# sssxyd/cpp-paddle-ocr

Measured on AMD Instinct MI355X. Metric: images/sec end-to-end (det+cls+rec) at 960x960, higher is better.
Workload: dtype f32

## Files before the change

### cpp-paddle-ocr_amd/binding.py

```python
import ctypes as C
import os

import numpy as np

HERE = os.path.dirname(os.path.abspath(__file__))
ROOT = os.path.dirname(HERE)
LIB_PATH = os.environ.get("OCR_LIB_PATH") or os.path.join(HERE, "lib", "libocr_hip.so")
MODELS = os.path.join(ROOT, "models")

_lib = None


class OcrError(RuntimeError):
    pass


class ocr_img(C.Structure):
    _fields_ = [("data", C.c_void_p), ("rows", C.c_int), ("cols", C.c_int), ("row_stride", C.c_size_t)]


class ocr_det_cfg(C.Structure):
    _fields_ = [("model_dir", C.c_char_p), ("device_id", C.c_int), ("limit_type", C.c_char_p),
                ("limit_side_len", C.c_int), ("det_db_thresh", C.c_double), ("det_db_box_thresh", C.c_double),
                ("det_db_unclip_ratio", C.c_double), ("det_db_score_mode", C.c_char_p), ("use_dilation", C.c_int),
# ... 778 lines not shown
            self.h = None


class Cls:
    def __init__(self, model_dir=None, device=0, cls_thresh=0.98, cls_batch_num=8, precision="fp32"):
        L = lib()
        _stage_protos(L)
        cfg = ocr_cls_cfg()
        L.ocr_cls_cfg_default(C.byref(cfg))
        self._keep = [(model_dir or os.path.join(MODELS, "cls")).encode(), precision.encode()]
        cfg.model_dir, cfg.precision = self._keep
        cfg.device_id, cfg.cls_thresh, cfg.cls_batch_num = device, cls_thresh, cls_batch_num
        self.h = C.c_void_p()
        check(L.ocr_cls_create(C.byref(cfg), C.byref(self.h)))
        self.times = (C.c_double * 3)()

    def run(self, crops):
        n = len(crops)
        labels = np.zeros(n, np.int32)
        scores = np.zeros(n, np.float32)
        if n:
            check(lib().ocr_cls_run(self.h, _imgs(crops), n, labels.ctypes.data, scores.ctypes.data, self.times))
        return labels, scores

    def probs(self, n):
        out = np.empty((n, 2), np.float32)
        check(lib().ocr_cls_probs(self.h, out.ctypes.data, out.size))
        return out

    def close(self):
        if self.h:
            lib().ocr_cls_destroy(self.h)
            self.h = None


class Rec:
    def __init__(self, model_dir=None, device=0, label_path=None, rec_batch_num=16, rec_img_h=28, rec_img_w=192,
                 precision="fp32", sort_mode=0):
        L = lib()
        _stage_protos(L)
        cfg = ocr_rec_cfg()
        L.ocr_rec_cfg_default(C.byref(cfg))
        md = model_dir or os.path.join(MODELS, "rec")
        self._keep = [md.encode(), (label_path or os.path.join(md, "ppocr_keys_v1.txt")).encode(), precision.encode()]
        cfg.model_dir, cfg.label_path, cfg.precision = self._keep
        cfg.device_id, cfg.rec_batch_num, cfg.rec_img_h, cfg.rec_img_w = device, rec_batch_num, rec_img_h, rec_img_w
        cfg.sort_mode = int(sort_mode)
        self.h = C.c_void_p()
        check(L.ocr_rec_create(C.byref(cfg), C.byref(self.h)))
        self.times = (C.c_double * 3)()

    def run(self, crops, max_len=512):
        n = len(crops)
        ids = np.zeros((n, max_len), np.int32)
        lens = np.zeros(n, np.int32)
        scores = np.zeros(n, np.float32)
        if n:
            check(lib().ocr_rec_run(self.h, _imgs(crops), n, ids.ctypes.data, max_len, lens.ctypes.data,
                                    scores.ctypes.data, self.times))
        return [ids[i, :lens[i]].copy() for i in range(n)], scores

    def run_chars(self, crops, max_len=512, topk=0):
        n = len(crops)
        ids = np.zeros((n, max_len), np.int32)
        lens = np.zeros(n, np.int32)
        scores = np.zeros(n, np.float32)
        steps = np.zeros((n, max_len), np.int32)
        nsteps = np.zeros((n, max_len), np.int32)
        probs = np.zeros((n, max_len), np.float32)
        geom = np.zeros((n, 3), np.int32)
        kk = max(int(topk), 1)
        alt_ids = np.zeros((n, max_len, kk), np.int32)
        alt_probs = np.zeros((n, max_len, kk), np.float32)
        if n:
            check(lib().ocr_rec_run_chars(self.h, _imgs(crops), n, ids.ctypes.data, max_len, lens.ctypes.data, scores.ctypes.data,
                                          steps.ctypes.data, nsteps.ctypes.data, probs.ctypes.data, geom.ctypes.data, int(topk),
                                          alt_ids.ctypes.data, alt_probs.ctypes.data, self.times))
        chars = []
        for i in range(n):
            m = lens[i]
            c = dict(steps=steps[i, :m].copy(), nsteps=nsteps[i, :m].copy(), probs=probs[i, :m].copy(), geom=tuple(int(v) for v in geom[i]))
            if topk > 0:
                c["alt_ids"] = alt_ids[i, :m].copy()
                c["alt_probs"] = alt_probs[i, :m].copy()
            chars.append(c)
        return [ids[i, :lens[i]].copy() for i in range(n)], scores, chars

    def logits_row(self, index, step):
        out = np.zeros(self.num_classes(), np.float32)
        check(lib().ocr_rec_logits_row(self.h, int(index), int(step), out.ctypes.data, out.size))
        return out

    def steps(self, index, cap=4096):
        amax = np.zeros(cap, np.int32)
        pmax = np.zeros(cap, np.float32)
        T = C.c_int()
        check(lib().ocr_rec_steps(self.h, index, amax.ctypes.data, pmax.ctypes.data, cap, C.byref(T)))
        return amax[:T.value].copy(), pmax[:T.value].copy()

    def set_launch_lines(self, n):
        check(lib().ocr_rec_set_launch_lines(self.h, int(n)))

    def timing(self, on=True):
        check(lib().ocr_rec_timing(self.h, int(on)))

    def timing_report(self):
        buf = C.create_string_buffer(1 << 20)
        check(lib().ocr_rec_timing_report(self.h, buf, len(buf)))
        out = {}
        for line in buf.value.decode().splitlines():
            name, ms, cnt, fl, by = line.split()
            out[name] = dict(ms=float(ms), count=int(cnt), flops=float(fl), bytes=float(by))
        return out

    def label(self, i):
        s = lib().ocr_rec_label(self.h, int(i))
        return s.decode("utf-8") if s is not None else None

    def text(self, ids):
        return "".join(self.label(i) for i in ids)

    def num_classes(self):
        return lib().ocr_rec_num_classes(self.h)

    def close(self):
        if self.h:
            lib().ocr_rec_destroy(self.h)
            self.h = None


class ocr_pipe_cfg(C.Structure):
    _fields_ = [("det", ocr_det_cfg), ("cls", ocr_cls_cfg), ("rec", ocr_rec_cfg), ("enable_cls", C.c_int),
                ("crop_mode", C.c_int), ("phases", C.c_int)]


class ocr_word(C.Structure):
    _fields_ = [("box", C.c_int32 * 8), ("ids_off", C.c_int32), ("ids_len", C.c_int32), ("confidence", C.c_float)]


class ocr_char(C.Structure):
    _fields_ = [("step", C.c_int32), ("nsteps", C.c_int32), ("prob", C.c_float), ("quad", C.c_int32 * 8)]


EXPORTS += ["ocr_pipe_cfg_default", "ocr_pipe_create", "ocr_pipe_destroy", "ocr_pipe_run", "ocr_pipe_run_chars", "ocr_pipe_run_device",
            "ocr_pipe_stage", "ocr_pipe_slot_probs", "ocr_pipe_run_staged", "ocr_pipe_run_device_on", "ocr_pipe_run_staged_on", "ocr_pipe_stage_jpeg", "ocr_jpeg_decode", "ocr_jpeg_time",
            "ocr_pipe_stage_jpeg_frames", "ocr_jpeg_decode_frame", "ocr_jpeg_time_frame", "ocr_pipe_slot_image",
            "ocr_png_decode", "ocr_png_time", "ocr_png_time_batch", "ocr_pipe_stage_coded",
            "ocr_raw_decode", "ocr_raw_time", "ocr_raw_time_batch", "ocr_pipe_stage_frames",
            "ocr_tiff_decode", "ocr_tiff_time", "ocr_tiff_time_batch", "ocr_pipe_stage_batch",
            "ocr_webp_decode", "ocr_webp_time", "ocr_webp_time_batch", "ocr_vp8_decode", "ocr_vp8_time", "ocr_vp8_time_batch", "ocr_j2k_decode", "ocr_j2k_time", "ocr_j2k_time_batch",
            "ocr_j2k_tier1", "ocr_j2k_decode_coded", "ocr_j2k_time_coded", "ocr_j2k_time_coded_batch",
            "ocr_tiff_expand", "ocr_tiff_decode_coded", "ocr_tiff_time_coded", "ocr_tiff_time_coded_batch",
            "ocr_tiff_inflate", "ocr_tiff_decode_deflate", "ocr_tiff_time_deflate", "ocr_tiff_time_deflate_batch",
            "ocr_pipe_label", "ocr_pipe_det_shape", "ocr_pipe_stats", "ocr_pipe_timing", "ocr_pipe_timing_filter", "ocr_pipe_timing_report", "ocr_dev_alloc",
            "ocr_dev_free", "ocr_dev_upload", "ocr_dev_download", "ocr_dev_sync", "ocr_dev_copy_time", "ocr_rotate_crop", "ocr_rotate_crop_shape", "ocr_rotate180_rois"]


def _pipe_protos(L):
    if getattr(L, "_pipe_protos_done", False):
        return
    _stage_protos(L)
    vp, ip = C.c_void_p, C.POINTER(C.c_int)
    L.ocr_pipe_cfg_default.argtypes = [C.POINTER(ocr_pipe_cfg)]
    L.ocr_pipe_create.argtypes = [C.POINTER(ocr_pipe_cfg), C.POINTER(vp)]
    L.ocr_pipe_destroy.argtypes = [vp]
    L.ocr_pipe_run.argtypes = [vp, C.POINTER(ocr_img), C.c_int, vp, C.c_int, vp, vp, vp, C.c_int, C.POINTER(C.c_double)]
    L.ocr_pipe_run_chars.argtypes = [vp, C.POINTER(ocr_img), C.c_int, vp, C.c_int, vp, vp, vp, C.c_int, vp, C.POINTER(C.c_double)]
    L.ocr_pipe_run_device.argtypes = [vp, vp, C.c_int, C.c_int, C.c_int, vp, vp, C.c_int, vp, vp, vp, C.c_int,
                                      C.POINTER(C.c_double)]
    L.ocr_pipe_stage.argtypes = [vp, C.c_int, C.POINTER(ocr_img), C.c_int]
    L.ocr_pipe_slot_probs.argtypes = [vp, C.c_int, vp, C.c_int]
    L.ocr_pipe_run_staged.argtypes = [vp, C.c_int, vp, C.c_int, vp, vp, vp, C.c_int, C.POINTER(C.c_double)]
    L.ocr_pipe_run_staged_on.argtypes = [vp, C.c_int, C.c_int, vp, C.c_int, vp, vp, vp, C.c_int, C.POINTER(C.c_double)]
    L.ocr_pipe_run_device_on.argtypes = [vp, C.c_int, vp, C.c_int, C.c_int, C.c_int, vp, vp, C.c_int, vp, vp, vp, C.c_int,
                                         C.POINTER(C.c_double)]
    L.ocr_pipe_label.argtypes = [vp, C.c_int]
    L.ocr_pipe_label.restype = C.c_char_p
    L.ocr_pipe_det_shape.argtypes = [vp, C.c_int, C.c_int, ip, ip]
    L.ocr_pipe_timing.argtypes = [vp, C.c_int]
    L.ocr_pipe_stats.argtypes = [vp, C.POINTER(C.c_longlong)]
    L.ocr_pipe_timing_report.argtypes = [vp, C.c_char_p, C.c_size_t]
    L.ocr_pipe_timing_filter.argtypes = [vp, C.c_char_p]
    L.ocr_dev_alloc.argtypes = [C.POINTER(vp), C.c_size_t]
    L.ocr_dev_free.argtypes = [vp]
    L.ocr_dev_upload.argtypes = [vp, vp, C.c_size_t]
    L.ocr_dev_download.argtypes = [vp, vp, C.c_size_t]
    L.ocr_rotate_crop.argtypes = [vp, C.c_int, C.c_int, C.c_size_t, vp, C.c_int, vp, C.c_size_t, vp, ip, ip]
    L.ocr_rotate_crop_shape.argtypes = [C.c_int, C.c_int, vp, ip, ip]
    L.ocr_rotate180_rois.argtypes = [vp, C.c_int, C.c_int, C.c_size_t, vp, C.c_int]
    L._pipe_protos_done = True


CROP_BOUNDING_RECT, CROP_ROTATE = 0, 1


class ocr_jpeg_comp(C.Structure):
    _fields_ = [("coef", C.c_void_p), ("quant", C.c_uint16 * 64), ("bw", C.c_int), ("bh", C.c_int), ("dw", C.c_int), ("dh", C.c_int)]


class ocr_jpeg_img(C.Structure):
    _fields_ = [("rows", C.c_int), ("cols", C.c_int), ("ncomp", C.c_int), ("hmax", C.c_int), ("vmax", C.c_int), ("orientation", C.c_int),
                ("comp", ocr_jpeg_comp * 3)]


class ocr_jpeg_fcomp(C.Structure):
    _fields_ = [("coef", C.c_void_p), ("quant", C.c_uint16 * 64), ("bw", C.c_int), ("bh", C.c_int), ("dw", C.c_int), ("dh", C.c_int),
                ("h", C.c_int), ("v", C.c_int)]


class ocr_jpeg_frame(C.Structure):
    _fields_ = [("rows", C.c_int), ("cols", C.c_int), ("ncomp", C.c_int), ("orientation", C.c_int), ("color", C.c_int), ("reserved", C.c_int),
                ("comp", ocr_jpeg_fcomp * 4)]


JPEG_COLORS = ["GREY", "YCBCR", "RGB", "CMYK", "YCCK"]


class JpegFrame:

    def __init__(self, rows, cols, color, orientation, comps):
        self.coefs = [np.ascontiguousarray(k["coef"], np.int16).reshape(-1).copy() for k in comps]
        c = ocr_jpeg_frame()
        c.rows, c.cols, c.ncomp, c.orientation, c.color = rows, cols, len(comps), orientation, color
        for o, k, coef in zip(c.comp, comps, self.coefs):
            o.coef = coef.ctypes.data
            o.quant[:] = [int(q) for q in np.asarray(k["quant"]).reshape(64)]
            o.bw, o.bh, o.dw, o.dh, o.h, o.v = (int(k[f]) for f in ("bw", "bh", "dw", "dh", "h", "v"))
        self.c = c

    def out_shape(self):
        return (self.c.cols, self.c.rows) if 5 <= self.c.orientation <= 8 else (self.c.rows, self.c.cols)

    def decode(self, device_id=0, fill=0, cap=None):
        return _decode_frame("ocr_jpeg_decode_frame", self.c, *self.out_shape(), device_id, fill, cap)

    def classic(self):
        c = self.c
        f = [(c.comp[i].h, c.comp[i].v) for i in range(c.ncomp)]
        if c.ncomp == 3 and (c.color != 1 or f[0] not in ((1, 1), (2, 1), (2, 2)) or f[1:] != [(1, 1), (1, 1)]):
            return None
        if c.ncomp not in (1, 3):
            return None
        im = ocr_jpeg_img()
        im.rows, im.cols, im.ncomp, im.orientation = c.rows, c.cols, c.ncomp, c.orientation
        im.hmax, im.vmax = f[0]
        for o, k in zip(im.comp, c.comp[:c.ncomp]):
            o.coef, o.bw, o.bh, o.dw, o.dh = k.coef, k.bw, k.bh, k.dw, k.dh
            C.memmove(o.quant, k.quant, 128)
        return im

    def decode_classic(self, device_id=0, fill=0):
        im = self.classic()
        return None if im is None else _decode_frame("ocr_jpeg_decode", im, *self.out_shape(), device_id, fill)


class ocr_png_segment(C.Structure):
    _fields_ = [("pass_", C.c_int32), ("first_row", C.c_int32), ("rows", C.c_int32)]


class ocr_png_frame(C.Structure):
    _fields_ = [("width", C.c_int), ("height", C.c_int), ("bit_depth", C.c_int), ("color_type", C.c_int), ("interlace", C.c_int),
                ("reserved", C.c_int), ("palette", C.c_uint8 * 768), ("data", C.c_void_p), ("data_len", C.c_size_t),
                ("segments", C.POINTER(ocr_png_segment)), ("nsegments", C.c_int)]


class PngFrame:

    def __init__(self, width, height, bit_depth, color_type, interlace, stream, segments, palette=None):
        self._data = np.frombuffer(bytes(stream), np.uint8).copy()
        self._segs = (ocr_png_segment * max(1, len(segments)))(*[ocr_png_segment(*s) for s in segments])
        c = ocr_png_frame()
        c.width, c.height, c.bit_depth, c.color_type, c.interlace = width, height, bit_depth, color_type, interlace
        if palette is not None:
            flat = np.asarray(palette, np.uint8).reshape(-1)
            C.memmove(c.palette, flat.ctypes.data, len(flat))
        c.data, c.data_len = self._data.ctypes.data, len(self._data)
        c.segments, c.nsegments = self._segs, len(segments)
        self.c = c

    def decode(self, device_id=0):
        return _decode_frame("ocr_png_decode", self.c, self.c.height, self.c.width, device_id)


class ocr_raw_frame(C.Structure):
    _fields_ = [("width", C.c_int), ("height", C.c_int), ("kind", C.c_int), ("bottom_up", C.c_int), ("row_stride", C.c_size_t),
                ("palette", C.c_uint8 * 1024), ("data", C.c_void_p), ("data_len", C.c_size_t)]


RAW_KINDS = ["INDEX1", "INDEX4", "INDEX8", "BGR555", "BGR565", "BGR24", "BGRX32", "RGB24", "GREY8", "GREY16BE", "RGB48BE", "BIT1_INV"]


class RawFrame:

    def __init__(self, width, height, kind, bottom_up, row_stride, rows, palette=None):
        self._data = np.frombuffer(bytes(rows), np.uint8).copy() if not isinstance(rows, np.ndarray) else np.ascontiguousarray(rows, np.uint8).reshape(-1).copy()
        c = ocr_raw_frame()
        c.width, c.height, c.kind, c.bottom_up, c.row_stride = width, height, kind, bottom_up, row_stride
        if palette is not None:
            flat = np.ascontiguousarray(palette, np.uint8).reshape(-1)
            C.memmove(c.palette, flat.ctypes.data, min(1024, len(flat)))
        c.data, c.data_len = self._data.ctypes.data, len(self._data)
        self.c = c

    def decode(self, device_id=0):
        return _decode_frame("ocr_raw_decode", self.c, self.c.height, self.c.width, device_id)


# ... 510 lines not shown
```

### cpp-paddle-ocr_amd/csrc/capi_net.hip

```cpp
#include <cstdio>
#include <atomic>
#include <cstring>
#include <mutex>
#include <vector>

#include "capi_common.h"
#include "plans_embedded.inc"

__attribute__((constructor)) static void ocr_runtime_env_defaults() { setenv("GPU_MAX_HW_QUEUES", "16", 0); }

namespace ocr {

const RtOptions& rt_options() {
  static RtOptions o;
  static std::once_flag once;
  std::call_once(once, [] {
    auto off = [](const char* n) { const char* e = getenv(n); return e && e[0] == '0'; };
    auto num = [](const char* n, long def) { const char* e = getenv(n); return e && *e ? atol(e) : def; };
    o.fuse = !off("OCR_FUSE");
    o.fuse_gap_min = num("OCR_FUSE_GAP_MIN", 64 * 1024);
    o.conv_small_nt = !off("OCR_CONV_SMALL_NT");
    o.conv_mt2 = !off("OCR_CONV_MT2");
    if (const char* e = getenv("OCR_CONV_MT2")) o.conv_mt2_force = e[0] == 'f';
    o.conv_c24 = !off("OCR_CONV_C24");
    { const char* e = getenv("OCR_DW_LDS"); o.dw_lds = !(e && e[0] == '0'); }
    { const char* e = getenv("OCR_DWPW2"); o.dwpw2 = !(e && e[0] == '0'); }
    { const char* e = getenv("OCR_XDW"); o.xdw = !(e && e[0] == '0'); }
    { const char* e = getenv("OCR_MFMA_X16"); o.mfma_x16 = !(e && e[0] == '0'); }
    { const char* e = getenv("OCR_ATTN_LINE"); o.attn_line = !(e && e[0] == '0'); }
    o.dwpw_items = (int)num("OCR_DWPW_ITEMS", 32);
    o.dwpw_force_upw = (int)num("OCR_DWPW_FORCE_UPW", 0);
    if (const char* e = getenv("OCR_DWPW_T4")) o.dwpw_t4_thin = e[0] == 't';
    o.trace_slice = (int)num("OCR_TRACE_SLICE", 0);
  });
  return o;
}
static std::mutex g_refuse_mu;
static std::string g_refuse;
static std::atomic<bool> g_refuse_on{false};
std::string rt_refuse_launch() {
  if (!g_refuse_on.load(std::memory_order_acquire)) return std::string();
  std::lock_guard<std::mutex> lk(g_refuse_mu);
  return g_refuse;
}
void rt_set_refuse_launch(const char* substr) {
  std::lock_guard<std::mutex> lk(g_refuse_mu);
  g_refuse = substr ? substr : "";
  g_refuse_on.store(!g_refuse.empty(), std::memory_order_release);
}

static std::atomic<int> g_wait_mode{-1};
int rt_wait_mode() {
  int m = g_wait_mode.load(std::memory_order_relaxed);
  if (m < 0) {
    const char* e = getenv("OCR_WAIT_MODE");
    m = e && e[0] == 's' ? 0 : 1;
    g_wait_mode.store(m, std::memory_order_relaxed);
  }
  return m;
}
void rt_set_wait_mode(int m) { g_wait_mode.store(m ? 1 : 0, std::memory_order_relaxed); }

std::shared_mutex& capture_mutex() {
  static std::shared_mutex m;
  return m;
}

static const std::vector<int>& device_map() {
  static std::vector<int> map;
  static std::once_flag once;
  std::call_once(once, [] {
    int n = 0;
    if (hipGetDeviceCount(&n) != hipSuccess) { (void)hipGetLastError(); n = 0; }
    if (const char* e = getenv("OCR_DEVICE_MAP")) {
      std::vector<int> m;
      bool ok = n > 0 && *e;
      for (const char* p = e; ok && *p;) {
        char* end = nullptr;
        const long v = strtol(p, &end, 10);
        ok = end != p && v >= 0 && v < n && m.size() < 64;
        if (ok) m.push_back((int)v);
        p = *end == ',' ? end + 1 : end;
        if (*end && *end != ',') ok = false;
      }
      if (ok && !m.empty()) { map = m; return; }
    }
    for (int i = 0; i < n; ++i) map.push_back(i);
  });
  return map;
}
static thread_local int g_logical_device = -1;
int rt_device_count() { return (int)device_map().size(); }
int rt_physical_device(int logical) { return logical >= 0 && logical < rt_device_count() ? device_map()[logical] : -1; }
int rt_current_device() { return g_logical_device; }
hipError_t rt_set_device(int logical) {
  const int phys = rt_physical_device(logical);
  if (phys < 0) return hipErrorInvalidDevice;
  const hipError_t e = hipSetDevice(phys);
  if (e == hipSuccess) g_logical_device = logical;
  return e;
}

static thread_local std::string g_last_error;
void set_last_error(const std::string& msg) { g_last_error = msg; }
int fail(int code, const std::string& msg) {
  g_last_error = msg;
  return code;
}

const char* embedded_plan(const char* kind) {
  if (!strcmp(kind, "det")) return kPlanDet;
  if (!strcmp(kind, "cls")) return kPlanCls;
  if (!strcmp(kind, "rec")) return kPlanRec;
  if (!strcmp(kind, "srv_det")) return kPlanSrv_det;
  if (!strcmp(kind, "srv_rec")) return kPlanSrv_rec;
  return nullptr;
}

bool load_model_dir(const std::string& model_dir, const char* weights_override, const char* kind, WeightMap& w, std::string& err) {
  std::string model;
  for (const char* n : {"/inference.pdmodel", "/model.pdmodel"})
    if (file_exists(model_dir + n)) { model = model_dir + n; break; }
  if (model.empty()) { err = "No valid model file found in " + model_dir; return false; }
  if (const char* plan = embedded_plan(kind)) {
    const char* po = strstr(plan, "graph_ops=");
    const char* pf = strstr(plan, "graph_fnv=");
    if (po && pf) {
      int nops = 0;
      unsigned long long fnv = 0;
      if (!pdmodel_graph_signature(model, nops, fnv, err)) return false;
      const int want_ops = atoi(po + 10);
      const unsigned long long want_fnv = strtoull(pf + 10, nullptr, 16);
      if (nops != want_ops || fnv != want_fnv) {
        char msg[320];
        snprintf(msg, sizeof msg, "%s is not the %s graph this library was built for (%d ops, signature %016llx; the plan expects %d, %016llx): "
                 "regenerate the plans with tools/make_plan.py and rebuild", model.c_str(), kind, nops, fnv, want_ops, want_fnv);
        err = msg;
        return false;
      }
    }
  }
  std::string params;
  if (weights_override) params = weights_override;
  else
    for (const char* n : {"/inference.pdiparams", "/model.pdiparams", "/synthetic.pdiparams"})
      if (file_exists(model_dir + n)) { params = model_dir + n; break; }
  if (params.empty() || !file_exists(params)) { err = "No parameter file found in " + model_dir; return false; }
  std::vector<std::string> names;
  if (!pdmodel_persistable_names(model, names, err)) return false;
  return pdiparams_read(params, names, w, err);
}

void priority_anchor(int device_id, int want) {
  static std::mutex mu;
  static hipStream_t anchor[64][2] = {};
  std::lock_guard<std::mutex> lk(mu);
  if (device_id < 0 || device_id >= 64) return;
  for (int k = 0; k < std::min(want, 2); ++k) {
    if (anchor[device_id][k]) continue;
    int least = 0, greatest = 0;
    if (hipDeviceGetStreamPriorityRange(&least, &greatest) != hipSuccess || least == greatest ||
        hipStreamCreateWithPriority(&anchor[device_id][k], hipStreamDefault, greatest) != hipSuccess) {
      anchor[device_id][k] = nullptr;
      (void)hipGetLastError();
      return;
    }
    (void)hipMemsetAsync(nullptr, 0, 0, anchor[device_id][k]);
    (void)hipGetLastError();
  }
}

}

using namespace ocr;

struct ocr_net {
  Net net;
  hipStream_t stream = nullptr;
  float* x_dev = nullptr;
  size_t x_cap = 0;
  int device = 0;
};

extern "C" {

const char* ocr_last_error(void) { return ocr::g_last_error.c_str(); }
// ... 279 lines not shown
```

### cpp-paddle-ocr_amd/csrc/hip_guard.h

```cpp
#pragma once
#include <hip/hip_runtime.h>

#include <mutex>
#include <shared_mutex>

namespace ocr {

std::shared_mutex& capture_mutex();
int rt_current_device();

template <class T>
inline hipError_t g_malloc(T** p, size_t bytes) {
  std::shared_lock<std::shared_mutex> lk(capture_mutex());
  return hipMalloc((void**)p, bytes);
}
inline hipError_t g_free(void* p) {
  std::shared_lock<std::shared_mutex> lk(capture_mutex());
  return hipFree(p);
}
inline hipError_t g_host_malloc(void** p, size_t bytes, unsigned flags) {
  std::shared_lock<std::shared_mutex> lk(capture_mutex());
  return hipHostMalloc(p, bytes, flags);
}
inline hipError_t g_host_free(void* p) {
  std::shared_lock<std::shared_mutex> lk(capture_mutex());
  return hipHostFree(p);
}
inline hipError_t g_memcpy(void* d, const void* s, size_t n, hipMemcpyKind k) {
  std::shared_lock<std::shared_mutex> lk(capture_mutex());
  return hipMemcpy(d, s, n, k);
}
inline hipError_t g_memcpy2d(void* d, size_t dp, const void* s, size_t sp, size_t w, size_t h, hipMemcpyKind k) {
  std::shared_lock<std::shared_mutex> lk(capture_mutex());
  return hipMemcpy2D(d, dp, s, sp, w, h, k);
}
inline hipError_t g_stream_create(hipStream_t* s) { return hipStreamCreateWithFlags(s, hipStreamNonBlocking); }

int rt_wait_mode();
void rt_set_wait_mode(int m);
inline hipError_t g_stream_sync(hipStream_t s) {
  if (rt_wait_mode() == 0) return hipStreamSynchronize(s);
  thread_local hipEvent_t ev[64] = {};
  const int d = rt_current_device();
  hipEvent_t& e = ev[d >= 0 && d < 64 ? d : 0];
  if (!e) {
    const hipError_t c = hipEventCreateWithFlags(&e, hipEventBlockingSync | hipEventDisableTiming);
    if (c != hipSuccess) { e = nullptr; (void)hipGetLastError(); return hipStreamSynchronize(s); }
  }
  const hipError_t r = hipEventRecord(e, s);
  if (r != hipSuccess) return r;
  return hipEventSynchronize(e);
}

hipError_t rt_set_device(int logical);
int rt_current_device();
int rt_physical_device(int logical);
int rt_device_count();

}
```

### cpp-paddle-ocr_amd/csrc/pipe.hip

```cpp
#include <algorithm>
#include <array>
#include <chrono>
#include <cstring>
#include <functional>
#include <map>
#include <memory>
#include <thread>

#include "capi_common.h"
#include "crop.h"
#include "frame_kinds.h"
#include "rot_groups.h"
#include "stages.h"

using namespace ocr;

namespace {
double now_ms() {
  return std::chrono::duration<double, std::milli>(std::chrono::steady_clock::now().time_since_epoch()).count();
}
}

using CharLists = std::vector<std::vector<ocr_char>>;
static int emit(const std::vector<std::vector<ocr_word>>& W, const std::vector<std::vector<int32_t>>& I, const std::vector<int>& order,
                ocr_word* words, int cap_words, int* word_off, int* nwords, int32_t* ids, int cap_ids, const CharLists* C = nullptr,
                ocr_char* chars = nullptr);

struct StageSlot {
  struct Img { int rows, cols, orig; size_t off, prob_off; };
  struct Group { int rows, cols, first, count; size_t off, prob_off; };
  PinnedStage pinned;
  DevBuf<uint8_t> dev;
  DevBuf<float> probs;
  std::vector<Img> imgs;
  std::vector<Group> groups;
  size_t bytes = 0, prob_floats = 0;
  bool has_probs = false, staged = false;
  hipEvent_t ready = nullptr;
  ~StageSlot() { if (ready) (void)hipEventDestroy(ready); }
};

static int rotate180_in_order(const std::vector<RotDesc>& rd, DevBuf<RotDesc>& scratch, DevBuf<int>& seg_scratch, hipStream_t stream,
                              std::string& err) {
  if (rd.empty()) return OCR_OK;
  const int n = (int)rd.size();
  std::vector<rot_groups::Rect> rects(n);
  std::vector<std::pair<const uint8_t*, size_t>> view(n);
  for (int k = 0; k < n; ++k) {
    rects[k] = rot_groups::Rect{rd[k].x, rd[k].y, rd[k].w, rd[k].h};
    view[k] = {rd[k].img, rd[k].stride};
  }
  std::vector<int> order, seg;
  rot_groups::group(rects, view, order, seg);
  std::vector<RotDesc> sorted;
  sorted.reserve(n);
  for (int k : order) sorted.push_back(rd[k]);
  if (!scratch.ensure(sorted.size(), err) || !seg_scratch.ensure(seg.size(), err)) return OCR_ERR_DEVICE;
  if (hipMemcpyAsync(scratch.p, sorted.data(), sorted.size() * sizeof(RotDesc), hipMemcpyHostToDevice, stream) != hipSuccess ||
      hipMemcpyAsync(seg_scratch.p, seg.data(), seg.size() * sizeof(int), hipMemcpyHostToDevice, stream) != hipSuccess) {
    err = "rotation list upload failed";
    return OCR_ERR_DEVICE;
  }
  launch_rotate180_groups(scratch.p, seg_scratch.p, (int)seg.size() - 1, stream);
  if (hipGetLastError() != hipSuccess) { err = "rotation launch failed"; return OCR_ERR_DEVICE; }
  return OCR_OK;
}

struct PipeWorker {
  DetStage det;
  std::vector<std::unique_ptr<DetStage>> det_extra;
  DetConfig det_cfg;
  int det_lanes = 8;
  bool det_ragged = true;
  bool det_post_ragged = true;
  RecStage rec;
  std::unique_ptr<ClsStage> cls;
  DevBuf<RotDesc> rot_desc;
  DevBuf<int> rot_seg;
  int crop_mode = 0;
  DevBuf<uint8_t> crop_arena;
  DevBuf<WarpDesc> warp_desc;
  std::vector<CropPlan> line_plan;
  std::vector<int32_t> boxes;
  std::vector<int> nbox;
  static constexpr int kCap = 1000;

  int create(const DetConfig& d, const RecConfig& r, const ClsConfig* k, int crop, std::string& err) {
    int code = 0;
    if (!det.create(d, err, code)) return code ? code : OCR_ERR_DEVICE;
    det_cfg = d;
    if (!rec.create(r, err, code)) return code ? code : OCR_ERR_DEVICE;
    rec.want_taps = false;
    if (k) {
      cls.reset(new ClsStage());
      if (!cls->create(*k, err, code)) return code ? code : OCR_ERR_DEVICE;
    }
    crop_mode = crop;
    return OCR_OK;
  }

  bool timing_on = false;
  std::string timing_filter;
  int add_det_extra(std::string& err) {
    std::unique_ptr<DetStage> d(new DetStage());
    int code = 0;
    if (!d->create(det_cfg, err, code)) return code ? code : OCR_ERR_DEVICE;
    d->net().set_timing_filter(timing_filter);
    d->net().enable_timing(timing_on);
    det_extra.push_back(std::move(d));
    return OCR_OK;
  }

  int run_images(uint8_t* base, const std::vector<StageSlot::Img>& imgs, const std::vector<StageSlot::Group>& groups, const float* probs,
                 std::vector<std::vector<ocr_word>>& out_words, std::vector<std::vector<int32_t>>& out_ids, double times[3], std::string& err,
                 CharLists* out_chars = nullptr) {
    const int count = (int)imgs.size();
    boxes.resize((size_t)count * kCap * 8);
    nbox.assign(count, 0);
    double t0 = now_ms();
    auto run_group = [&](DetStage& d, const StageSlot::Group& g, std::string& e) {
      const size_t row = (size_t)g.cols * 3, img_bytes = row * g.rows;
      return d.run_device(base + g.off, img_bytes, row, g.rows, g.cols, g.count, boxes.data() + (size_t)g.first * kCap * 8, kCap,
                          nbox.data() + g.first, nullptr, e, probs ? probs + g.prob_off : nullptr);
    };
    const bool srv_det = det.srv() != nullptr;
    const int lanes = srv_det ? 1 : (int)std::min<size_t>((size_t)det_lanes, groups.size());
    if (groups.size() > 1 && det_ragged && !srv_det) {
      std::vector<DetStage::MixedGroup> mg(groups.size());
      std::vector<size_t> gpx(groups.size());
      for (size_t gi = 0; gi < groups.size(); ++gi) {
        const auto& g = groups[gi];
        mg[gi] = DetStage::MixedGroup{g.rows, g.cols, g.count, g.off, g.prob_off};
        int rh = 0, rw = 0;
        { float a, b; DetStage::resize_shape(g.rows, g.cols, det.cfg().limit_type, det.cfg().limit_side_len, rh, rw, a, b); }
        gpx[gi] = (size_t)g.count * rh * rw;
      }
      static const size_t budget = [] { const char* e = getenv("OCR_DET_CHUNK_MP"); return (size_t)(e && atoi(e) > 0 ? atoi(e) : 64) << 20; }();
      std::vector<std::pair<size_t, size_t>> chunks;
      for (size_t g0 = 0; g0 < groups.size();) {
        size_t g1 = g0, px = 0;
        while (g1 < groups.size() && (g1 == g0 || px + gpx[g1] <= budget)) px += gpx[g1++];
        chunks.emplace_back(g0, g1);
        g0 = g1;
      }
      const int want_extra = std::max(lanes - 1, chunks.size() > 1 ? 1 : 0);
      while ((int)det_extra.size() < want_extra) {
        int rc = add_det_extra(err);
        if (rc) return rc;
      }
      const int ninst = 1 + (int)det_extra.size();
      auto net_stage = [&](size_t k) -> DetStage& { return (k & 1) && ninst > 1 ? *det_extra[0] : det; };
      auto start = [&](size_t k) {
        return net_stage(k).mixed_net(base, mg.data() + chunks[k].first, (int)(chunks[k].second - chunks[k].first), probs, err);
      };
      int rc = start(0);
      if (rc) return rc;
      for (size_t k = 0; k < chunks.size(); ++k) {
        const size_t g0 = chunks[k].first, g1 = chunks[k].second;
        DetStage& src = net_stage(k);
        const bool more = k + 1 < chunks.size();
        if (more) {
          rc = start(k + 1);
          if (rc) return rc;
        }
        if (!det.cfg().use_dilation && det_post_ragged) {
          const auto& gf = groups[g0];
          rc = src.post_mixed(mg.data() + g0, (int)(g1 - g0), boxes.data() + (size_t)gf.first * kCap * 8, kCap, nbox.data() + gf.first, err);
          if (rc) return rc;
          src.collect_timings();
          continue;
        }
        DetStage* busy = more ? &net_stage(k + 1) : nullptr;
        std::vector<DetStage*> post;
        for (int l = 0; l < ninst; ++l) {
          DetStage* d = l == 0 ? &det : det_extra[l - 1].get();
          if (d != busy) post.push_back(d);
        }
        const int np = (int)post.size();
        std::vector<int> rcs(np, OCR_OK);
        std::vector<std::string> errs(np);
        auto lane_fn = [&](int l) {
          DetStage& d = *post[l];
          for (size_t gi = g0 + l; gi < g1; gi += np) {
            const auto& g = groups[gi];
            rcs[l] = d.post_group(src.mixed_prob((int)(gi - g0)), src.mixed_bitmap((int)(gi - g0)), mg[gi], &d == &src ? nullptr : src.done(),
                                  boxes.data() + (size_t)g.first * kCap * 8, kCap, nbox.data() + g.first, errs[l]);
            if (rcs[l]) return;
          }
        };
        std::vector<std::thread> th;
        for (int l = 1; l < np; ++l) th.emplace_back(lane_fn, l);
        lane_fn(0);
        for (auto& t : th) t.join();
        for (int l = 0; l < np; ++l)
          if (rcs[l]) { err = errs[l]; return rcs[l]; }
        if (g_stream_sync(src.stream()) != hipSuccess) { err = "det stream sync failed"; return OCR_ERR_DEVICE; }
        src.collect_timings();
      }
    } else if (lanes <= 1) {
      for (const auto& g : groups) {
        int rc = run_group(det, g, err);
        if (rc) return rc;
      }
    } else {
      while ((int)det_extra.size() < lanes - 1) {
        int rc = add_det_extra(err);
        if (rc) return rc;
      }
      if (g_stream_sync(det.stream()) != hipSuccess) { err = "det stream sync failed"; return OCR_ERR_DEVICE; }
      std::vector<int> rcs(lanes, OCR_OK);
      std::vector<std::string> errs(lanes);
      auto lane_fn = [&](int l) {
        DetStage& d = l == 0 ? det : *det_extra[l - 1];
        for (size_t gi = l; gi < groups.size(); gi += lanes) {
          rcs[l] = run_group(d, groups[gi], errs[l]);
          if (rcs[l]) return;
        }
      };
      std::vector<std::thread> th;
      for (int l = 1; l < lanes; ++l) th.emplace_back(lane_fn, l);
      lane_fn(0);
      for (auto& t : th) t.join();
      for (int l = 0; l < lanes; ++l)
        if (rcs[l]) { err = errs[l]; return rcs[l]; }
    }
    double t1 = now_ms();
    times[0] += t1 - t0;
    std::vector<LineSrc> lines;
    std::vector<int> seg(1, 0);
    std::vector<int> line_box;
    line_plan.clear();
    if (crop_mode == OCR_CROP_ROTATE) {
      int rc = rotate_crops(base, imgs, lines, seg, line_box, err);
      if (rc) return rc;
    } else
    for (int i = 0; i < count; ++i) {
      const int rows = imgs[i].rows, cols = imgs[i].cols;
      const size_t row = (size_t)cols * 3;
      for (int j = 0; j < nbox[i]; ++j) {
        const int32_t* b = &boxes[((size_t)i * kCap + j) * 8];
        int x0 = b[0], x1 = b[0], y0 = b[1], y1 = b[1];
        for (int k = 1; k < 4; ++k) {
          x0 = std::min(x0, b[2 * k]); x1 = std::max(x1, b[2 * k]);
          y0 = std::min(y0, b[2 * k + 1]); y1 = std::max(y1, b[2 * k + 1]);
        }
        const int ix0 = std::max(x0, 0), iy0 = std::max(y0, 0);
        const int ix1 = std::min(x1 + 1, cols), iy1 = std::min(y1 + 1, rows);
        if (ix1 - ix0 > 0 && iy1 - iy0 > 0) {
          line_box.push_back((int)lines.size() - seg.back());
          lines.push_back(LineSrc{base + imgs[i].off, row, ix0, iy0, ix1 - ix0, iy1 - iy0});
        }
      }
      seg.push_back((int)lines.size());
    }
    out_words.assign(count, {});
    out_ids.assign(count, {});
    if (out_chars) out_chars->assign(count, {});
    if (lines.empty()) return OCR_OK;
    std::vector<int> labels;
    if (cls) {
      labels.resize(lines.size());
      std::vector<float> scores(lines.size());
      int rc = cls->run_lines(lines, labels.data(), scores.data(), err);
      if (rc) return rc;
      std::vector<RotDesc> rd;
      for (size_t k = 0; k < lines.size(); ++k)
        if (labels[k] == 1) rd.push_back(RotDesc{const_cast<uint8_t*>(lines[k].img), lines[k].stride, lines[k].x, lines[k].y, lines[k].w, lines[k].h});
      int rrc = rotate180_in_order(rd, rot_desc, rot_seg, cls->stream(), err);
      if (rrc) return rrc;
      if (g_stream_sync(cls->stream()) != hipSuccess) { err = "cls stream sync failed"; return OCR_ERR_DEVICE; }
    }
    double t2 = now_ms();
    times[1] += t2 - t1;
    const int max_len = 256;
    std::vector<int32_t> ids(lines.size() * max_len);
    std::vector<int> lens(lines.size());
    std::vector<float> scores(lines.size());
    std::vector<int32_t> csteps, cnsteps, geom;
    std::vector<float> cprobs;
    int rc;
    if (out_chars) {
      csteps.resize(ids.size()); cnsteps.resize(ids.size()); cprobs.resize(ids.size()); geom.resize(lines.size() * 3);
      RecStage::CharOut co;
      co.steps = csteps.data(); co.nsteps = cnsteps.data(); co.probs = cprobs.data(); co.geom = geom.data();
      rc = rec.run_lines_chars(lines, seg, ids.data(), max_len, lens.data(), scores.data(), co, err);
    } else {
      rc = rec.run_lines(lines, seg, ids.data(), max_len, lens.data(), scores.data(), err);
    }
    if (rc) return rc;
    times[2] += now_ms() - t2;
    for (int i = 0; i < count; ++i) {
      for (int k = seg[i]; k < seg[i + 1]; ++k) {
        ocr_word w;
        memcpy(w.box, &boxes[((size_t)i * kCap + line_box[k]) * 8], sizeof(w.box));
        w.ids_off = (int32_t)out_ids[i].size();
        w.ids_len = lens[k];
        w.confidence = scores[k];
        out_ids[i].insert(out_ids[i].end(), ids.begin() + (size_t)k * max_len, ids.begin() + (size_t)k * max_len + lens[k]);
        out_words[i].push_back(w);
        if (out_chars)
          for (int j = 0; j < lens[k]; ++j) {
            const size_t q = (size_t)k * max_len + j;
            ocr_char ch;
            ch.step = csteps[q]; ch.nsteps = cnsteps[q]; ch.prob = cprobs[q];
            const LineSrc& L = lines[k];
            char_quad(ch.step, ch.nsteps, geom[3 * k], geom[3 * k + 1], geom[3 * k + 2], L.w, L.h, !labels.empty() && labels[k] == 1,
                      crop_mode == OCR_CROP_ROTATE ? &line_plan[k] : nullptr, L.x, L.y, imgs[i].rows, imgs[i].cols, ch.quad);
            (*out_chars)[i].push_back(ch);
          }
      }
    }
    return OCR_OK;
  }

  int rotate_crops(const uint8_t* base, const std::vector<StageSlot::Img>& imgs, std::vector<LineSrc>& lines, std::vector<int>& seg,
                   std::vector<int>& line_box, std::string& err) {
    std::vector<WarpDesc> wd;
    std::vector<size_t> off;
    size_t total = 0;
    int max_px = 0;
    for (int i = 0; i < (int)imgs.size(); ++i) {
      const int rows = imgs[i].rows, cols = imgs[i].cols;
      const size_t row = (size_t)cols * 3;
      for (int j = 0; j < nbox[i]; ++j) {
        CropPlan p;
        if (!plan_rotate_crop(rows, cols, &boxes[((size_t)i * kCap + j) * 8], p)) continue;
        WarpDesc d;
        d.src = base + imgs[i].off + (size_t)p.top * row + (size_t)p.left * 3;
        d.sstride = row; d.sw = p.sw; d.sh = p.sh; d.dst = nullptr; d.dw = p.dw; d.dh = p.dh; d.rot = p.rot; d.bw0 = p.bw0;
        memcpy(d.m, p.minv, sizeof(d.m));
        wd.push_back(d);
        off.push_back(total);
        total += ((size_t)p.dw * p.dh * 3 + 15) & ~(size_t)15;
        max_px = std::max(max_px, p.dw * p.dh);
        line_box.push_back(j);
        line_plan.push_back(p);
        lines.push_back(LineSrc{nullptr, (size_t)p.ocols * 3, 0, 0, p.ocols, p.orows});
      }
      seg.push_back((int)lines.size());
    }
    if (wd.empty()) return OCR_OK;
    if (!crop_arena.ensure(total, err) || !warp_desc.ensure(wd.size(), err)) return OCR_ERR_DEVICE;
    for (size_t k = 0; k < wd.size(); ++k) {
      wd[k].dst = crop_arena.p + off[k];
      lines[k].img = wd[k].dst;
    }
    if (hipMemcpyAsync(warp_desc.p, wd.data(), wd.size() * sizeof(WarpDesc), hipMemcpyHostToDevice, det.stream()) != hipSuccess) {
      err = "crop list upload failed";
      return OCR_ERR_DEVICE;
    }
    launch_warp_crops(warp_desc.p, (int)wd.size(), max_px, det.stream());
    if (g_stream_sync(det.stream()) != hipSuccess) { err = "crop kernel failed"; return OCR_ERR_DEVICE; }
    return OCR_OK;
  }
};

struct ocr_pipe {
  PipeWorker w0;
  std::vector<std::unique_ptr<PipeWorker>> extra;
  int phases = 2;
  int parts_per_chain = 1;
  int device = 0;
  StageSlot slots[2];
  hipStream_t copy_stream = nullptr;
  FrameScratch frame_scratch;
  DevBuf<uint8_t> work;
  DevBuf<uint8_t> work_chain[4];
  PipeWorker* worker(int c) { return c == 0 ? &w0 : (c >= 1 && c <= (int)extra.size() ? extra[c - 1].get() : nullptr); }

  ~ocr_pipe() { if (copy_stream) (void)hipStreamDestroy(copy_stream); }

  int layout(StageSlot& S, int count, const std::function<void(int, int&, int&)>& size_of, std::string& err) {
    if (!copy_stream && hipStreamCreateWithFlags(&copy_stream, hipStreamNonBlocking) != hipSuccess) { err = "hipStreamCreate failed"; return OCR_ERR_DEVICE; }
    if (!S.ready && hipEventCreateWithFlags(&S.ready, hipEventDisableTiming) != hipSuccess) { err = "hipEventCreate failed"; return OCR_ERR_DEVICE; }
    if (S.staged && hipEventSynchronize(S.ready) != hipSuccess) { err = "staging event failed"; return OCR_ERR_DEVICE; }
    S.staged = false;
    std::vector<int> order(count), rows(count), cols(count);
    for (int i = 0; i < count; ++i) { order[i] = i; size_of(i, rows[i], cols[i]); }
    std::stable_sort(order.begin(), order.end(), [&](int a, int b) { return rows[a] != rows[b] ? rows[a] < rows[b] : cols[a] < cols[b]; });
    const std::vector<StageSlot::Img> before = S.imgs;
    S.imgs.clear();
    S.groups.clear();
    size_t off = 0, poff = 0;
    for (int k = 0; k < count; ++k) {
      const int r = rows[order[k]], c = cols[order[k]];
      if (S.groups.empty() || S.groups.back().rows != r || S.groups.back().cols != c) {
        off = (off + 255) & ~(size_t)255;
        S.groups.push_back({r, c, k, 0, off, poff});
      }
      S.groups.back().count++;
      int rh = 0, rw = 0;
      { float a, b; DetStage::resize_shape(r, c, w0.det.cfg().limit_type, w0.det.cfg().limit_side_len, rh, rw, a, b); }
      S.imgs.push_back({r, c, order[k], off, poff});
      off += (size_t)r * c * 3;
      poff += (size_t)rh * rw;
    }
    S.bytes = off;
    S.prob_floats = poff;
    bool same = before.size() == S.imgs.size();
    for (size_t k = 0; same && k < before.size(); ++k)
      same = before[k].rows == S.imgs[k].rows && before[k].cols == S.imgs[k].cols && before[k].orig == S.imgs[k].orig;
    if (!same) S.has_probs = false;
    if (!S.dev.ensure(off + 256, err)) return OCR_ERR_DEVICE;
    return OCR_OK;
  }

  int stage(int si, const ocr_img* imgs, int count, std::string& err) {
    StageSlot& S = slots[si];
    int rc = layout(S, count, [&](int i, int& r, int& c) { r = imgs[i].rows; c = imgs[i].cols; }, err);
    if (rc) return rc;
    const size_t off = S.bytes;
    if (!S.pinned.reserve(off, err)) return OCR_ERR_DEVICE;
    parallel_copy((size_t)count, off, [&](size_t k) {
      const ocr_img& im = imgs[S.imgs[k].orig];
      const size_t row = (size_t)im.cols * 3, stride = im.row_stride ? im.row_stride : row;
      uint8_t* dst = S.pinned.p + S.imgs[k].off;
      if (stride == row) memcpy(dst, im.data, row * im.rows);
      else for (int y = 0; y < im.rows; ++y) memcpy(dst + row * y, im.data + stride * y, row);
    });
    if (hipMemcpyAsync(S.dev.p, S.pinned.p, off, hipMemcpyHostToDevice, copy_stream) != hipSuccess) { err = "H2D copy failed"; return OCR_ERR_DEVICE; }
    if (hipEventRecord(S.ready, copy_stream) != hipSuccess) { err = "hipEventRecord failed"; return OCR_ERR_DEVICE; }
    S.staged = true;
    return OCR_OK;
  }

  int stage_coded(int si, const ocr_coded_frame* frames, int count, std::string& err) {
    StageSlot& S = slots[si];
    int rc = layout(S, count, [&](int i, int& r, int& c) { kFrameKinds[frames[i].kind].size(frames[i].frame, r, c); }, err);
    if (rc) return rc;
    struct Bucket {
      std::vector<const void*> frames;
      std::vector<uint8_t*> dst;
      std::vector<int> ids;
    } bucket[kFrameKindCount];
    for (const StageSlot::Img& im : S.imgs) {
      Bucket& b = bucket[frames[im.orig].kind];
      b.frames.push_back(frames[im.orig].frame);
      b.dst.push_back(S.dev.p + im.off);
      b.ids.push_back(im.orig);
    }
    for (int kind : kFrameLaunchOrder) {
      const Bucket& b = bucket[kind];
      if (b.frames.empty()) continue;
      rc = kFrameKinds[kind].decode(b.frames.data(), (int)b.frames.size(), b.dst.data(), frame_scratch, copy_stream, err, b.ids.data());
      if (rc) return rc;
    }
    if (hipEventRecord(S.ready, copy_stream) != hipSuccess) { err = "hipEventRecord failed"; return OCR_ERR_DEVICE; }
    S.staged = true;
    return OCR_OK;
  }

  int slot_probs(int si, const float* const* probs, int count, std::string& err) {
    StageSlot& S = slots[si];
    if (!S.staged || count != (int)S.imgs.size()) { err = "stage the slot's images first (same count)"; return OCR_ERR_ARG; }
    if (!S.probs.ensure(S.prob_floats + 64, err)) return OCR_ERR_DEVICE;
    for (int k = 0; k < count; ++k) {
      const size_t n = (k + 1 < count ? S.imgs[k + 1].prob_off : S.prob_floats) - S.imgs[k].prob_off;
      const hipError_t e = hipMemcpyAsync(S.probs.p + S.imgs[k].prob_off, probs[S.imgs[k].orig], n * sizeof(float), hipMemcpyDefault, copy_stream);
      if (e != hipSuccess) {
        err = std::string("probability map upload failed: ") + hipGetErrorString(e);
        return OCR_ERR_DEVICE;
      }
    }
    if (hipEventRecord(S.ready, copy_stream) != hipSuccess) { err = "hipEventRecord failed"; return OCR_ERR_DEVICE; }
    S.has_probs = true;
    return OCR_OK;
  }

  int run_images(uint8_t* base, const std::vector<StageSlot::Img>& imgs, const std::vector<StageSlot::Group>& groups, const float* probs,
                 std::vector<std::vector<ocr_word>>& out_words, std::vector<std::vector<int32_t>>& out_ids, double times[3], std::string& err,
                 CharLists* out_chars = nullptr) {
    const int count = (int)imgs.size();
    const int nchains = (int)std::min<size_t>(1 + extra.size(), (size_t)count);
    if (nchains < 2) return w0.run_images(base, imgs, groups, probs, out_words, out_ids, times, err, out_chars);
    const int K = (int)std::min<size_t>((size_t)nchains * parts_per_chain, (size_t)count);
    std::vector<std::vector<StageSlot::Img>> pi(K);
    std::vector<std::vector<StageSlot::Group>> pg(K);
    std::vector<std::vector<int>> gidx(K);
    std::vector<size_t> load(K, 0);
    auto give = [&](int p, const StageSlot::Group& g, int first, int n) {
      int rh = 0, rw = 0;
      { float a, b; DetStage::resize_shape(g.rows, g.cols, w0.det.cfg().limit_type, w0.det.cfg().limit_side_len, rh, rw, a, b); }
      StageSlot::Group ng = g;
      ng.first = (int)pi[p].size();
      ng.count = n;
      ng.off = g.off + (size_t)first * g.rows * g.cols * 3;
      ng.prob_off = g.prob_off + (size_t)first * rh * rw;
      pg[p].push_back(ng);
      for (int k = 0; k < n; ++k) { pi[p].push_back(imgs[g.first + first + k]); gidx[p].push_back(g.first + first + k); }
      load[p] += (size_t)n * g.rows * g.cols;
    };
    size_t total = 0;
    for (const auto& g : groups) total += (size_t)g.count * g.rows * g.cols;
    const size_t share = (total + K - 1) / K;
    for (const auto& g : groups) {
      const size_t px = (size_t)g.rows * g.cols;
      int first = 0;
      while (first < g.count) {
        const int p = (int)(std::min_element(load.begin(), load.end()) - load.begin());
        const int left = g.count - first;
        const size_t room = share > load[p] ? share - load[p] : 0;
        int n = left;
        if ((size_t)left * px > room + px / 2) n = (int)std::min<size_t>(left, std::max<size_t>(1, (room + px / 2) / px));
        give(p, g, first, n);
        first += n;
      }
    }
    if (g_stream_sync(w0.det.stream()) != hipSuccess) { err = "det stream sync failed"; return OCR_ERR_DEVICE; }
    std::vector<std::vector<std::vector<ocr_word>>> W(K);
    std::vector<std::vector<std::vector<int32_t>>> I(K);
    std::vector<CharLists> Ch(K);
    std::vector<std::array<double, 3>> t(K, std::array<double, 3>{0, 0, 0});
    std::vector<int> rc(K, OCR_OK);
    std::vector<std::string> errs(K);
    auto chain = [&](int c) {
      PipeWorker& w = c == 0 ? w0 : *extra[c - 1];
      for (int p = c; p < K; p += nchains) {
        if (pi[p].empty()) continue;
        rc[p] = w.run_images(base, pi[p], pg[p], probs, W[p], I[p], t[p].data(), errs[p], out_chars ? &Ch[p] : nullptr);
        if (rc[p]) return;
      }
    };
    std::vector<std::thread> th;
    for (int c = 1; c < nchains; ++c) th.emplace_back([&, c]() { (void)rt_set_device(device); chain(c); });
    chain(0);
    for (auto& x : th) x.join();
    for (int p = 0; p < K; ++p)
      if (rc[p]) { err = errs[p]; return rc[p]; }
    out_words.assign(count, {});
    out_ids.assign(count, {});
    if (out_chars) out_chars->assign(count, {});
    for (int p = 0; p < K; ++p)
      for (size_t k = 0; k < gidx[p].size(); ++k) {
        out_words[gidx[p][k]] = std::move(W[p][k]);
        out_ids[gidx[p][k]] = std::move(I[p][k]);
        if (out_chars) (*out_chars)[gidx[p][k]] = std::move(Ch[p][k]);
      }
    for (int k = 0; k < 3; ++k) {
      double m = 0;
      for (int c = 0; c < nchains; ++c) {
        double sum = 0;
        for (int p = c; p < K; p += nchains) sum += t[p][k];
        m = std::max(m, sum);
      }
      times[k] += m;
    }
    return OCR_OK;
  }

  int run_slot(int si, ocr_word* words, int cap_words, int* word_off, int* nwords, int32_t* ids, int cap_ids, double times[3], int chain = -1,
               ocr_char* chars = nullptr) {
    StageSlot& S = slots[si];
    if (!S.staged || S.imgs.empty()) return fail(OCR_ERR_ARG, "nothing staged in this slot");
    std::string err;
    PipeWorker* one = chain >= 0 ? worker(chain) : nullptr;
    if (chain >= 0 && !one) return fail(OCR_ERR_ARG, "no such chain (0 <= chain < phases)");
    PipeWorker& first = one ? *one : w0;
    DevBuf<uint8_t>& clone = one ? work_chain[chain] : work;
    if (hipStreamWaitEvent(first.det.stream(), S.ready, 0) != hipSuccess) return fail(OCR_ERR_DEVICE, "hipStreamWaitEvent failed");
    if (!clone.ensure(S.bytes + 256, err)) return fail(OCR_ERR_DEVICE, err);
    if (hipMemcpyAsync(clone.p, S.dev.p, S.bytes, hipMemcpyDeviceToDevice, first.det.stream()) != hipSuccess) return fail(OCR_ERR_DEVICE, "clone failed");
    double t[3] = {0, 0, 0};
    std::vector<std::vector<ocr_word>> W;
    std::vector<std::vector<int32_t>> I;
    CharLists C;
    CharLists* pc = chars ? &C : nullptr;
    const int rc = one ? one->run_images(clone.p, S.imgs, S.groups, S.has_probs ? S.probs.p : nullptr, W, I, t, err, pc)
                       : run_images(clone.p, S.imgs, S.groups, S.has_probs ? S.probs.p : nullptr, W, I, t, err, pc);
    if (rc) return fail(rc, err);
    if (times) { times[0] = t[0]; times[1] = t[1]; times[2] = t[2]; }
    const int count = (int)S.imgs.size();
    std::vector<int> order(count);
    for (int k = 0; k < count; ++k) order[S.imgs[k].orig] = k;
    return emit(W, I, order, words, cap_words, word_off, nwords, ids, cap_ids, pc, chars);
  }
};

static int emit(const std::vector<std::vector<ocr_word>>& W, const std::vector<std::vector<int32_t>>& I, const std::vector<int>& order,
                ocr_word* words, int cap_words, int* word_off, int* nwords, int32_t* ids, int cap_ids, const CharLists* C, ocr_char* chars) {
  int wo = 0, io = 0;
  for (size_t i = 0; i < order.size(); ++i) {
    const auto& w = W[order[i]];
    const auto& d = I[order[i]];
    word_off[i] = wo;
    nwords[i] = (int)w.size();
    if (wo + (int)w.size() > cap_words || io + (int)d.size() > cap_ids) return fail(OCR_ERR_CAPACITY, "result buffers too small");
    for (size_t k = 0; k < w.size(); ++k) {
      words[wo + k] = w[k];
      words[wo + k].ids_off += io;
    }
    if (!d.empty()) memcpy(ids + io, d.data(), d.size() * sizeof(int32_t));
    if (C && chars && !d.empty()) memcpy(chars + io, (*C)[order[i]].data(), d.size() * sizeof(ocr_char));
    wo += (int)w.size();
    io += (int)d.size();
  }
  return OCR_OK;
}

extern "C" {

void ocr_pipe_cfg_default(ocr_pipe_cfg* c) {
  if (!c) return;
  memset(c, 0, sizeof(*c));
  ocr_det_cfg_default(&c->det);
  ocr_cls_cfg_default(&c->cls);
  ocr_rec_cfg_default(&c->rec);
  c->enable_cls = 0;
  c->crop_mode = OCR_CROP_BOUNDING_RECT;
}

int ocr_pipe_create(const ocr_pipe_cfg* c, ocr_pipe** out) {
  if (!c || !out || !c->det.model_dir || !c->rec.model_dir || !c->rec.label_path) return fail(OCR_ERR_ARG, "null argument");
  if (c->enable_cls && !c->cls.model_dir) return fail(OCR_ERR_ARG, "cls model_dir missing");
  std::unique_ptr<ocr_pipe> h(new ocr_pipe());
  h->device = c->det.device_id;
  if (c->crop_mode != OCR_CROP_BOUNDING_RECT && c->crop_mode != OCR_CROP_ROTATE) return fail(OCR_ERR_ARG, "unknown crop_mode");
  if (c->phases < 0 || c->phases > 4) return fail(OCR_ERR_ARG, "phases must be 0 (default) or 1..4");
  h->phases = c->phases ? c->phases : 2;
  if (const char* e = getenv("OCR_PIPE_PHASES")) h->phases = std::min(4, std::max(1, atoi(e)));
  std::string err;
  DetConfig d;
  d.model_dir = c->det.model_dir; d.device = c->det.device_id;
  if (c->det.limit_type) d.limit_type = c->det.limit_type;
  d.limit_side_len = c->det.limit_side_len; d.thresh = c->det.det_db_thresh; d.box_thresh = c->det.det_db_box_thresh;
  d.unclip_ratio = c->det.det_db_unclip_ratio;
  if (c->det.det_db_score_mode) d.score_mode = c->det.det_db_score_mode;
  d.use_dilation = c->det.use_dilation;
  if (c->det.precision) d.precision = c->det.precision;
  d.max_batch = c->det.max_batch > 0 ? c->det.max_batch : 1;
  d.cv_compat = resolve_cv_compat(c->det.cv_compat);
  RecConfig r;
  r.model_dir = c->rec.model_dir; r.label_path = c->rec.label_path; r.device = c->det.device_id;
  r.batch_num = c->rec.rec_batch_num; r.img_h = c->rec.rec_img_h; r.img_w = c->rec.rec_img_w; r.sort_mode = c->rec.sort_mode;
  if (c->rec.precision) r.precision = c->rec.precision;
  ClsConfig k;
  if (c->enable_cls) {
    k.model_dir = c->cls.model_dir; k.device = c->det.device_id; k.thresh = c->cls.cls_thresh;
    k.batch_num = c->cls.cls_batch_num > 0 ? c->cls.cls_batch_num : 1;
    if (c->cls.precision) k.precision = c->cls.precision;
  }
  int lanes = 8;
  if (const char* e = getenv("OCR_DET_LANES")) lanes = std::min(32, std::max(1, atoi(e)));
  int rc = h->w0.create(d, r, c->enable_cls ? &k : nullptr, c->crop_mode, err);
  if (rc) return fail(rc, err);
  h->w0.det_lanes = lanes;
  for (int p = 1; p < h->phases; ++p) {
    h->extra.emplace_back(new PipeWorker());
    rc = h->extra.back()->create(d, r, c->enable_cls ? &k : nullptr, c->crop_mode, err);
    if (rc) return fail(rc, err);
  }
  h->w0.det_lanes = std::max(1, (lanes + h->phases - 1) / h->phases);
  for (auto& w : h->extra) w->det_lanes = h->w0.det_lanes;
  if (const char* e = getenv("OCR_DET_RAGGED")) {
    h->w0.det_ragged = e[0] != '0';
    h->w0.det_post_ragged = e[0] != 'n';
    for (auto& w : h->extra) { w->det_ragged = h->w0.det_ragged; w->det_post_ragged = h->w0.det_post_ragged; }
  }
  priority_anchor(h->device, 2);
  *out = h.release();
  return OCR_OK;
}
void ocr_pipe_destroy(ocr_pipe* h) { delete h; }

static int pipe_run_device(ocr_pipe* h, int chain, const void* dev_bgr, int rows, int cols, int count, const float* dev_prob, ocr_word* words,
                           int cap_words, int* word_off, int* nwords, int32_t* ids, int cap_ids, double times[3]) {
  if (!h || !dev_bgr || rows <= 0 || cols <= 0 || count < 1 || !words || !word_off || !nwords || !ids)
    return fail(OCR_ERR_ARG, "bad argument");
  CAPI_HIP(rt_set_device(h->device));
  PipeWorker* one = chain >= 0 ? h->worker(chain) : nullptr;
  if (chain >= 0 && !one) return fail(OCR_ERR_ARG, "no such chain (0 <= chain < phases)");
  PipeWorker& first = one ? *one : h->w0;
  DevBuf<uint8_t>& clone = one ? h->work_chain[chain] : h->work;
  double t[3] = {0, 0, 0};
  std::vector<std::vector<ocr_word>> W;
  std::vector<std::vector<int32_t>> I;
  std::string err;
  const size_t img_bytes = (size_t)rows * cols * 3, bytes = img_bytes * count;
  if (!clone.ensure(bytes + 256, err)) return fail(OCR_ERR_DEVICE, err);
  CAPI_HIP(hipMemcpyAsync(clone.p, dev_bgr, bytes, hipMemcpyDeviceToDevice, first.det.stream()));
  std::vector<StageSlot::Img> imgs(count);
  for (int i = 0; i < count; ++i) imgs[i] = {rows, cols, i, img_bytes * i, 0};
  const std::vector<StageSlot::Group> groups = {{rows, cols, 0, count, 0, 0}};
  const int rc = one ? one->run_images(clone.p, imgs, groups, dev_prob, W, I, t, err) : h->run_images(clone.p, imgs, groups, dev_prob, W, I, t, err);
  if (rc) return fail(rc, err);
  if (times) { times[0] = t[0]; times[1] = t[1]; times[2] = t[2]; }
  std::vector<int> order(count);
  for (int i = 0; i < count; ++i) order[i] = i;
  return emit(W, I, order, words, cap_words, word_off, nwords, ids, cap_ids);
}
int ocr_pipe_run_device(ocr_pipe* h, const void* dev_bgr, int rows, int cols, int count, const float* dev_prob, ocr_word* words,
                        int cap_words, int* word_off, int* nwords, int32_t* ids, int cap_ids, double times[3]) {
  return pipe_run_device(h, -1, dev_bgr, rows, cols, count, dev_prob, words, cap_words, word_off, nwords, ids, cap_ids, times);
}
int ocr_pipe_run_device_on(ocr_pipe* h, int chain, const void* dev_bgr, int rows, int cols, int count, const float* dev_prob,
                           ocr_word* words, int cap_words, int* word_off, int* nwords, int32_t* ids, int cap_ids, double times[3]) {
  if (chain < 0) return fail(OCR_ERR_ARG, "no such chain (0 <= chain < phases)");
  return pipe_run_device(h, chain, dev_bgr, rows, cols, count, dev_prob, words, cap_words, word_off, nwords, ids, cap_ids, times);
}

static bool stage_args_ok(const ocr_pipe* h, bool images, int slot, int count) { return h && images && count >= 1 && (slot == 0 || slot == 1); }

static int stage_validated(ocr_pipe* h, int slot, const std::vector<ocr_coded_frame>& frames) {
  CAPI_HIP(rt_set_device(h->device));
  std::string err;
  const int rc = h->stage_coded(slot, frames.data(), (int)frames.size(), err);
  return rc ? fail(rc, err) : OCR_OK;
}
static std::vector<ocr_coded_frame> tagged(const ocr_jpeg_frame* frames, int count) {
  std::vector<ocr_coded_frame> t((size_t)count);
  for (int i = 0; i < count; ++i) t[i] = ocr_coded_frame{OCR_FRAME_JPEG, frames + i};
  return t;
}

int ocr_pipe_stage(ocr_pipe* h, int slot, const ocr_img* imgs, int count) {
  if (!stage_args_ok(h, imgs, slot, count)) return fail(OCR_ERR_ARG, "bad argument");
  for (int i = 0; i < count; ++i)
    if (!imgs[i].data || imgs[i].rows <= 0 || imgs[i].cols <= 0) return fail(OCR_ERR_ARG, "Empty image data provided");
  CAPI_HIP(rt_set_device(h->device));
  std::string err;
  const int rc = h->stage(slot, imgs, count, err);
  return rc ? fail(rc, err) : OCR_OK;
}

int ocr_pipe_stage_jpeg(ocr_pipe* h, int slot, const ocr_jpeg_img* imgs, int count) {
  if (!stage_args_ok(h, imgs, slot, count)) return fail(OCR_ERR_ARG, "bad argument");
  for (int i = 0; i < count; ++i)
    if (!jpeg_img_valid(imgs[i])) return fail(OCR_ERR_ARG, "bad JPEG coefficient descriptor");
  std::vector<ocr_jpeg_frame> frames((size_t)count);
  for (int i = 0; i < count; ++i) {
    frames[i] = jpeg_frame_of(imgs[i]);
    if (const char* fault = jpeg_frame_fault(frames[i])) return fail(OCR_ERR_ARG, fault);
  }
  return stage_validated(h, slot, tagged(frames.data(), count));
}

int ocr_pipe_stage_jpeg_frames(ocr_pipe* h, int slot, const ocr_jpeg_frame* frames, int count) {
  if (!stage_args_ok(h, frames, slot, count)) return fail(OCR_ERR_ARG, "bad argument");
  for (int i = 0; i < count; ++i)
    if (const char* fault = jpeg_frame_fault(frames[i])) return fail(OCR_ERR_ARG, fault);
  return stage_validated(h, slot, tagged(frames, count));
}

int ocr_pipe_stage_frames(ocr_pipe* h, int slot, const ocr_jpeg_frame* const* jpegs, const ocr_png_frame* const* pngs,
                          const ocr_raw_frame* const* raws, int count) {
  if (!stage_args_ok(h, jpegs || pngs || raws, slot, count)) return fail(OCR_ERR_ARG, "bad argument");
  std::vector<ocr_coded_frame> t((size_t)count);
  for (int i = 0; i < count; ++i) {
    const ocr_jpeg_frame* j = jpegs ? jpegs[i] : nullptr;
    const ocr_png_frame* p = pngs ? pngs[i] : nullptr;
    const ocr_raw_frame* r = raws ? raws[i] : nullptr;
    if ((j != nullptr) + (p != nullptr) + (r != nullptr) != 1)
      return fail(OCR_ERR_ARG, raws ? "every image is a JPEG frame, a PNG frame or a raw frame: exactly one of the three"
                                    : "every image is a JPEG frame or a PNG frame, not both and not neither");
    if (const char* fault = j ? jpeg_frame_fault(*j) : p ? png_frame_fault(*p) : raw_frame_fault(*r)) return fail(OCR_ERR_ARG, fault);
    t[i] = j ? ocr_coded_frame{OCR_FRAME_JPEG, j} : p ? ocr_coded_frame{OCR_FRAME_PNG, p} : ocr_coded_frame{OCR_FRAME_RAW, r};
  }
  return stage_validated(h, slot, t);
}

int ocr_pipe_stage_batch(ocr_pipe* h, int slot, const ocr_coded_frame* frames, int count) {
  if (!stage_args_ok(h, frames, slot, count)) return fail(OCR_ERR_ARG, "bad argument");
  for (int i = 0; i < count; ++i) {
    const void* f = frames[i].frame;
    if (!f) return fail(OCR_ERR_ARG, "null frame in the batch");
    const int kind = frames[i].kind;
    const char* fault = kind >= 0 && kind < kFrameKindCount ? kFrameKinds[kind].fault(f) : "frame kind is not an ocr_frame_kind";
    if (fault) return fail(OCR_ERR_ARG, fault);
  }
  return stage_validated(h, slot, std::vector<ocr_coded_frame>(frames, frames + count));
}

int ocr_pipe_stage_coded(ocr_pipe* h, int slot, const ocr_jpeg_frame* const* jpegs, const ocr_png_frame* const* pngs, int count) {
  return ocr_pipe_stage_frames(h, slot, jpegs, pngs, nullptr, count);
}

int ocr_pipe_slot_image(ocr_pipe* h, int slot, int index, uint8_t* bgr, size_t cap, int* rows, int* cols) {
  if (!h || !bgr || !rows || !cols || slot < 0 || slot > 1) return fail(OCR_ERR_ARG, "bad argument");
  StageSlot& S = h->slots[slot];
  if (!S.staged) return fail(OCR_ERR_ARG, "nothing is staged in the slot");
  for (const StageSlot::Img& im : S.imgs) {
    if (im.orig != index) continue;
    const size_t bytes = (size_t)im.rows * im.cols * 3;
    if (bytes > cap) return fail(OCR_ERR_CAPACITY, "output buffer too small");
    CAPI_HIP(rt_set_device(h->device));
    CAPI_HIP(hipEventSynchronize(S.ready));
    CAPI_HIP(g_memcpy(bgr, S.dev.p + im.off, bytes, hipMemcpyDeviceToHost));
    *rows = im.rows; *cols = im.cols;
    return OCR_OK;
  }
  return fail(OCR_ERR_ARG, "no staged image with that index");
}

int ocr_pipe_slot_probs(ocr_pipe* h, int slot, const float* const* probs, int count) {
  if (!h || !probs || count < 1 || slot < 0 || slot > 1) return fail(OCR_ERR_ARG, "bad argument");
  for (int i = 0; i < count; ++i) if (!probs[i]) return fail(OCR_ERR_ARG, "null probability map");
  CAPI_HIP(rt_set_device(h->device));
  std::string err;
  const int rc = h->slot_probs(slot, probs, count, err);
  return rc ? fail(rc, err) : OCR_OK;
}

int ocr_pipe_run_staged(ocr_pipe* h, int slot, ocr_word* words, int cap_words, int* word_off, int* nwords, int32_t* ids,
                        int cap_ids, double times[3]) {
  if (!h || slot < 0 || slot > 1 || !words || !word_off || !nwords || !ids) return fail(OCR_ERR_ARG, "bad argument");
  CAPI_HIP(rt_set_device(h->device));
  return h->run_slot(slot, words, cap_words, word_off, nwords, ids, cap_ids, times);
}

int ocr_pipe_run_staged_on(ocr_pipe* h, int chain, int slot, ocr_word* words, int cap_words, int* word_off, int* nwords, int32_t* ids,
                           int cap_ids, double times[3]) {
  if (!h || chain < 0 || slot < 0 || slot > 1 || !words || !word_off || !nwords || !ids) return fail(OCR_ERR_ARG, "bad argument");
  CAPI_HIP(rt_set_device(h->device));
  return h->run_slot(slot, words, cap_words, word_off, nwords, ids, cap_ids, times, chain);
}

int ocr_pipe_run(ocr_pipe* h, const ocr_img* imgs, int count, ocr_word* words, int cap_words, int* word_off, int* nwords,
                 int32_t* ids, int cap_ids, double times[3]) {
  if (!h || !imgs || count < 1 || !words || !word_off || !nwords || !ids) return fail(OCR_ERR_ARG, "bad argument");
  const int rc = ocr_pipe_stage(h, 0, imgs, count);
  if (rc) return rc;
  return h->run_slot(0, words, cap_words, word_off, nwords, ids, cap_ids, times);
}

int ocr_pipe_run_chars(ocr_pipe* h, const ocr_img* imgs, int count, ocr_word* words, int cap_words, int* word_off, int* nwords,
                       int32_t* ids, int cap_ids, ocr_char* chars, double times[3]) {
  if (!h || !imgs || count < 1 || !words || !word_off || !nwords || !ids || !chars) return fail(OCR_ERR_ARG, "bad argument");
  const int rc = ocr_pipe_stage(h, 0, imgs, count);
  if (rc) return rc;
  return h->run_slot(0, words, cap_words, word_off, nwords, ids, cap_ids, times, -1, chars);
}

const char* ocr_pipe_label(ocr_pipe* h, int id) {
  if (!h || id < 0 || id >= (int)h->w0.rec.labels().size()) return nullptr;
  return h->w0.rec.labels()[id].c_str();
}

int ocr_pipe_det_shape(ocr_pipe* h, int rows, int cols, int* net_rows, int* net_cols) {
  if (!h || !net_rows || !net_cols) return fail(OCR_ERR_ARG, "null argument");
  float a, b;
  DetStage::resize_shape(rows, cols, h->w0.det.cfg().limit_type, h->w0.det.cfg().limit_side_len, *net_rows, *net_cols, a, b);
  return OCR_OK;
}

static std::vector<Net*> pipe_nets(ocr_pipe* h) {
  std::vector<Net*> v;
  std::vector<PipeWorker*> ws{&h->w0};
  for (auto& w : h->extra) ws.push_back(w.get());
  for (PipeWorker* w : ws) {
    v.push_back(&w->det.net());
    for (auto& d : w->det_extra) v.push_back(&d->net());
    if (w->cls) v.push_back(&w->cls->net());
    v.push_back(&w->rec.net());
  }
  return v;
}
static std::vector<SrvNet*> pipe_srv_nets(ocr_pipe* h) {
  std::vector<SrvNet*> v;
  std::vector<PipeWorker*> ws{&h->w0};
  for (auto& w : h->extra) ws.push_back(w.get());
  for (PipeWorker* w : ws) {
    if (w->det.srv()) v.push_back(w->det.srv());
    if (w->rec.srv()) v.push_back(w->rec.srv());
  }
  return v;
}
int ocr_pipe_timing(ocr_pipe* h, int enable) {
  if (!h) return fail(OCR_ERR_ARG, "null handle");
  for (Net* net : pipe_nets(h)) {
    net->enable_timing(enable != 0);
    net->reset_timings();
  }
  for (SrvNet* net : pipe_srv_nets(h)) {
    net->enable_timing(enable != 0);
    net->reset_timings();
  }
  h->w0.timing_on = enable != 0;
  for (auto& w : h->extra) w->timing_on = enable != 0;
  return OCR_OK;
}
int ocr_pipe_stats(ocr_pipe* h, long long out[3]) {
  if (!h || !out) return fail(OCR_ERR_ARG, "null argument");
  out[0] = out[1] = out[2] = 0;
  auto add = [&](Net& n) { out[0] += n.stats().runs; out[1] += n.stats().binds; out[2] += n.stats().graph_replays; };
  std::vector<PipeWorker*> ws{&h->w0};
  for (auto& w : h->extra) ws.push_back(w.get());
  for (PipeWorker* w : ws) {
    add(w->det.net());
    for (auto& d : w->det_extra) add(d->net());
    if (w->cls) add(w->cls->net());
    add(w->rec.net());
  }
  return OCR_OK;
}
int ocr_pipe_timing_filter(ocr_pipe* h, const char* substr) {
  if (!h) return fail(OCR_ERR_ARG, "null handle");
  const std::string f = substr ? substr : "";
  for (Net* net : pipe_nets(h)) net->set_timing_filter(f);
  h->w0.timing_filter = f;
  for (auto& w : h->extra) w->timing_filter = f;
  return OCR_OK;
}
int ocr_pipe_timing_report(ocr_pipe* h, char* buf, size_t cap) {
  if (!h || !buf) return fail(OCR_ERR_ARG, "null argument");
  size_t off = 0;
  std::map<std::string, KernelTiming> all;
  for (Net* net : pipe_nets(h))
    for (auto& kv : net->timings()) {
      KernelTiming& t = all[kv.first];
      t.ms += kv.second.ms; t.count += kv.second.count; t.flops += kv.second.flops; t.bytes += kv.second.bytes;
    }
  {
    std::vector<PipeWorker*> ws{&h->w0};
    for (auto& w : h->extra) ws.push_back(w.get());
    for (PipeWorker* w : ws)
      for (int k = 0; k < 2; ++k) {
        SrvNet* net = k ? w->rec.srv() : w->det.srv();
        if (!net) continue;
        for (auto& kv : net->timings()) {
          KernelTiming& t = all[std::string(k ? "rec." : "det.") + kv.first];
          t.ms += kv.second.ms; t.count += kv.second.count; t.flops += kv.second.flops; t.bytes += kv.second.bytes;
        }
      }
  }
  for (auto& kv : all) {
    int n = snprintf(buf + off, cap > off ? cap - off : 0, "%s %.6f %ld %.0f %.0f\n", kv.first.c_str(), kv.second.ms,
                     kv.second.count, kv.second.flops, kv.second.bytes);
    if (n < 0 || off + n >= cap) return fail(OCR_ERR_CAPACITY, "report buffer too small");
    off += n;
  }
  if (off < cap) buf[off] = 0;
  return OCR_OK;
}

int ocr_rotate_crop_shape(int rows, int cols, const int32_t* box, int* out_rows, int* out_cols) {
  if (!box || !out_rows || !out_cols) return fail(OCR_ERR_ARG, "null argument");
  CropPlan p;
  if (!plan_rotate_crop(rows, cols, box, p)) return fail(OCR_ERR_ARG, "box has no crop inside the image");
  *out_rows = p.orows;
  *out_cols = p.ocols;
  return OCR_OK;
}

int ocr_rotate_crop(const uint8_t* bgr, int rows, int cols, size_t row_stride, const int32_t* boxes, int n, uint8_t* out,
                    size_t out_cap, size_t* out_off, int* out_rows, int* out_cols) {
  if (!bgr || rows <= 0 || cols <= 0 || !boxes || n < 1 || !out || !out_off || !out_rows || !out_cols)
    return fail(OCR_ERR_ARG, "bad argument");
  const size_t row = (size_t)cols * 3, stride = row_stride ? row_stride : row;
  std::vector<WarpDesc> wd(n);
  std::vector<size_t> src_off(n);
  size_t total = 0;
  int max_px = 0;
  for (int k = 0; k < n; ++k) {
    CropPlan p;
    if (!plan_rotate_crop(rows, cols, boxes + 8 * k, p)) return fail(OCR_ERR_ARG, "box has no crop inside the image");
    WarpDesc& d = wd[k];
    d.sstride = row; d.sw = p.sw; d.sh = p.sh; d.dw = p.dw; d.dh = p.dh; d.rot = p.rot; d.bw0 = p.bw0;
    src_off[k] = (size_t)p.top * row + (size_t)p.left * 3;
    memcpy(d.m, p.minv, sizeof(d.m));
    out_off[k] = total;
    out_rows[k] = p.orows;
    out_cols[k] = p.ocols;
    total += (size_t)p.dw * p.dh * 3;
    max_px = std::max(max_px, p.dw * p.dh);
  }
  out_off[n] = total;
  if (total > out_cap) return fail(OCR_ERR_CAPACITY, "crop buffer too small");
  std::string err;
  DevBuf<uint8_t> dimg, dout;
  DevBuf<WarpDesc> ddesc;
  if (!dimg.ensure(row * rows, err) || !dout.ensure(total, err) || !ddesc.ensure(n, err)) return fail(OCR_ERR_DEVICE, err);
  for (int k = 0; k < n; ++k) {
    wd[k].src = dimg.p + src_off[k];
    wd[k].dst = dout.p + out_off[k];
  }
  CAPI_HIP(g_memcpy2d(dimg.p, row, bgr, stride, row, rows, hipMemcpyHostToDevice));
  CAPI_HIP(g_memcpy(ddesc.p, wd.data(), n * sizeof(WarpDesc), hipMemcpyHostToDevice));
  launch_warp_crops(ddesc.p, n, max_px, 0);
  CAPI_HIP(hipGetLastError());
  CAPI_HIP(g_memcpy(out, dout.p, total, hipMemcpyDeviceToHost));
  return OCR_OK;
}

int ocr_rotate180_rois(uint8_t* bgr, int rows, int cols, size_t row_stride, const int32_t* rects, int n) {
  if (!bgr || rows <= 0 || cols <= 0 || !rects || n < 1) return fail(OCR_ERR_ARG, "bad argument");
  const size_t row = (size_t)cols * 3, stride = row_stride ? row_stride : row;
  std::string err;
  DevBuf<uint8_t> dimg;
  DevBuf<RotDesc> ddesc;
  DevBuf<int> dseg;
  if (!dimg.ensure(row * rows, err)) return fail(OCR_ERR_DEVICE, err);
  std::vector<RotDesc> rd(n);
  for (int k = 0; k < n; ++k) {
    const int32_t* r = rects + 4 * k;
    if (r[0] < 0 || r[1] < 0 || r[2] < 1 || r[3] < 1 || r[0] + r[2] > cols || r[1] + r[3] > rows) return fail(OCR_ERR_ARG, "rectangle outside the image");
    rd[k] = RotDesc{dimg.p, row, r[0], r[1], r[2], r[3]};
  }
  CAPI_HIP(g_memcpy2d(dimg.p, row, bgr, stride, row, rows, hipMemcpyHostToDevice));
  const int rc = rotate180_in_order(rd, ddesc, dseg, 0, err);
  if (rc) return fail(rc, err);
  CAPI_HIP(g_memcpy2d(bgr, stride, dimg.p, row, row, rows, hipMemcpyDeviceToHost));
  return OCR_OK;
}

int ocr_dev_alloc(void** p, size_t bytes) {
  if (!p) return fail(OCR_ERR_ARG, "null argument");
  CAPI_HIP(g_malloc(p, bytes));
  return OCR_OK;
}
int ocr_dev_free(void* p) { CAPI_HIP(g_free(p)); return OCR_OK; }
int ocr_dev_upload(void* dst, const void* src, size_t bytes) { CAPI_HIP(g_memcpy(dst, src, bytes, hipMemcpyHostToDevice)); return OCR_OK; }
int ocr_dev_download(void* dst, const void* src, size_t bytes) { CAPI_HIP(g_memcpy(dst, src, bytes, hipMemcpyDeviceToHost)); return OCR_OK; }
int ocr_dev_sync(void) { CAPI_HIP(hipDeviceSynchronize()); return OCR_OK; }

}
```

### cpp-paddle-ocr_amd/csrc/rt_options.h

```cpp
#pragma once
#include <string>

namespace ocr {

struct RtOptions {
  bool fuse = true;
  long fuse_gap_min = 65536;
  bool conv_small_nt = true;
  bool conv_mt2 = true;
  bool conv_mt2_force = false;
  bool conv_c24 = true;
  bool attn_line = true;
  bool mfma_x16 = true;
  bool dw_lds = true;
  bool xdw = true;
  bool dwpw2 = true;
  int dwpw_items = 32;
  int dwpw_force_upw = 0;
  bool dwpw_t4_thin = false;
  int trace_slice = 0;
};
const RtOptions& rt_options();

std::string rt_refuse_launch();
void rt_set_refuse_launch(const char* substr);

}
```

### cpp-paddle-ocr_amd/csrc/stages.h

```cpp
#pragma once
#include <hip/hip_runtime.h>

#include <memory>
#include <string>
#include <vector>

#include "../../include/ocr_hip.h"
#include "kernels_post.h"
#include "kernels_pre.h"
#include "net.h"
#include "srv_net.h"

namespace ocr {

template <class T>
struct DevBuf {
  T* p = nullptr;
  size_t cap = 0;
  ~DevBuf() { if (p) (void)g_free(p); }
  bool ensure(size_t n, std::string& err) {
    if (n <= cap) return true;
    if (p) (void)g_free(p);
    p = nullptr;
    cap = 0;
    hipError_t e = g_malloc(&p, n * sizeof(T));
    if (e != hipSuccess) { err = std::string("hipMalloc: ") + hipGetErrorString(e); return false; }
    cap = n;
    return true;
  }
};

struct StageTimer {
  hipEvent_t ev[4] = {nullptr, nullptr, nullptr, nullptr};
  bool init(std::string& err);
  ~StageTimer();
  void mark(int i, hipStream_t s) { (void)hipEventRecord(ev[i], s); }
  void read(double times[3]);
};

struct DetConfig {
  std::string model_dir, limit_type = "max", score_mode = "fast", precision = "fp32";
  int device = 0, limit_side_len = 512, use_dilation = 0, max_batch = 1;
  double thresh = 0.2, box_thresh = 0.4, unclip_ratio = 1.8;
  int cv_compat = 410;
};

class DetStage {
 public:
  ~DetStage();
  bool create(const DetConfig& cfg, std::string& err, int& code);
  int run(const ocr_img* imgs, int count, int32_t* boxes, int cap, int* n, double times[3], std::string& err);
  int run_device(const uint8_t* dev_imgs, size_t img_bytes, size_t stride, int rows, int cols, int count, int32_t* boxes,
                 int cap, int* n, double times[3], std::string& err, const float* prob_override = nullptr);
  struct MixedGroup { int rows, cols, count; size_t off, prob_off; };
  int mixed_net(const uint8_t* base, const MixedGroup* groups, int ngroups, const float* prob_override, std::string& err);
  const float* mixed_prob(int gi) const { return mixed_probs_[gi]; }
  const uint8_t* mixed_bitmap(int gi) const { return bitmap_.p + mixed_pix_[gi]; }
  hipEvent_t done() const { return mixed_done_; }
  void collect_timings() { net_.collect_timings(); }
  int post_mixed(const MixedGroup* groups, int ngroups, int32_t* boxes, int cap, int* n, std::string& err);
  int post_group(const float* prob, const uint8_t* bitmap, const MixedGroup& g, hipEvent_t wait_for, int32_t* boxes, int cap, int* n,
                 std::string& err);
  uint8_t* dev_images_mut() { return src_.p; }
  int post_only(const float* prob, int rows, int cols, int src_rows, int src_cols, int32_t* boxes, int cap, int* n,
                std::string& err);
  int post_stages(ocr_post_stages* out, std::string& err);
  const uint8_t* dev_images() const { return src_.p; }
  size_t dev_image_bytes() const { return (size_t)src_rows_ * src_cols_ * 3; }
  hipStream_t stream() const { return stream_; }
  Net& net() { return net_; }
  int last_count = 0, last_h = 0, last_w = 0;
  const float* prob_dev() const { return srv_ ? (const float*)srv_->tensor_ptr(srv_->output_tid()) : net_.tensor_ptr(net_.output_tid()); }
  SrvNet* srv() { return srv_.get(); }
  const uint8_t* bitmap_dev() const { return cfg_.use_dilation ? bitmap2_.p : bitmap_.p; }
  const uint8_t* resized_dev() const { return resized_.p; }
  const DetConfig& cfg() const { return cfg_; }
  static void resize_shape(int h, int w, const std::string& limit_type, int limit_side_len, int& rh, int& rw,
                           float& ratio_h, float& ratio_w);

 private:
  bool ensure_post(int count, size_t px, int H, int W, int cap, std::string& err);
  int post_launch(PostArgs a, int count, int32_t* boxes, int cap, int* n, std::string& err);
  int run_post(int count, int H, int W, const float* prob, float ratio_h, float ratio_w, int src_h, int src_w,
               int32_t* boxes, int cap, int* n, std::string& err, const uint8_t* bitmap = nullptr);
  std::vector<size_t> mixed_pix_;
  const float* mixed_prob_base_ = nullptr;
  DevBuf<PostImg> post_img_;
  std::vector<const float*> mixed_probs_;
  hipEvent_t mixed_done_ = nullptr;
  DetConfig cfg_;
  Net net_;
  std::unique_ptr<SrvNet> srv_;
  hipStream_t stream_ = nullptr;
  StageTimer timer_;
  DevBuf<float> lut_, x_, prob_in_;
  DevBuf<uint8_t> src_, resized_, bitmap_, bitmap2_, touch_;
  DevBuf<int> labels_, chunk_cnt_, ncont_all_, ncont_, starts_, npts_, poff_, iscratch_, cand_boxes_, cand_valid_, status_, out_boxes_,
      out_n_;
  DevBuf<unsigned long long> pool_;
  DevBuf<unsigned> mask_pool_, mask_top_;
  DevBuf<float> stage_rec_;
  bool tap_armed_ = false, tap_valid_ = false;
  int tap_h_ = 0, tap_w_ = 0;
  DevBuf<int> pool_need_;
  size_t mask_words_ = 0;
  static size_t mask_words(int H, int W) { return (((size_t)H * W / 4 + (1u << 16)) + 31) & ~(size_t)31; }
  int src_rows_ = 0, src_cols_ = 0;
  int ithresh_ = 0;
  int pool_cap_ = 0;
  int bm_n_ = 0;
};

struct LineSrc {
  const uint8_t* img;
  size_t stride;
  int x, y, w, h;
};

struct RecConfig {
  std::string model_dir, label_path, precision = "fp32";
  int device = 0, batch_num = 16, img_h = 28, img_w = 192;
  int sort_mode = 0;
};

class RecStage {
 public:
  ~RecStage();
  struct CharOut {
    int32_t* steps = nullptr;
    int32_t* nsteps = nullptr;
    float* probs = nullptr;
    int32_t* geom = nullptr;
    int topk = 0;
    int32_t* alt_ids = nullptr;
    float* alt_probs = nullptr;
  };
  bool create(const RecConfig& cfg, std::string& err, int& code);
  int run(const ocr_img* imgs, int n, int32_t* ids, int max_len, int* lens, float* scores, double times[3],
          std::string& err);
  int run_lines(const std::vector<LineSrc>& lines, const std::vector<int>& seg, int32_t* ids, int max_len, int* lens,
                float* scores, std::string& err, const CharOut* co = nullptr);
  int run_chars(const ocr_img* imgs, int n, int32_t* ids, int max_len, int* lens, float* scores, const CharOut& co, double times[3],
                std::string& err);
  int run_lines_chars(const std::vector<LineSrc>& lines, const std::vector<int>& seg, int32_t* ids, int max_len, int* lens,
                      float* scores, const CharOut& co, std::string& err) {
    return run_lines(lines, seg, ids, max_len, lens, scores, err, &co);
  }
  int logits_row(int index, int step, float* out, size_t cap_floats, std::string& err);
  bool want_taps = true;
  static constexpr int kSrvLinesPerLaunch = 1024;
  static_assert((unsigned long long)kSrvLinesPerLaunch * (12 * 80 * 768) * sizeof(float) < 0xfffffff0ull, "a server launch passes the buffer-descriptor guard");
  int max_lines_per_launch = 4096;
  const std::vector<std::string>& labels() const { return labels_; }
  hipStream_t stream() const { return stream_; }
  Net& net() { return net_; }
  SrvNet* srv() { return srv_.get(); }
  std::vector<int> tap_T, tap_off;
  std::vector<int> tap_amax;
  std::vector<float> tap_pmax;

 private:
  struct LinesCtx;
  RecConfig cfg_;
  Net net_;
  std::unique_ptr<SrvNet> srv_;
  hipStream_t stream_ = nullptr;
  StageTimer timer_;
  std::vector<std::string> labels_;
  DevBuf<float> lut_, pmax_, scores_, x_;
  DevBuf<int> amax_, ids_, lens_;
  DevBuf<uint8_t> staging_;
  DevBuf<LineDesc> descs_;
  DevBuf<int> csteps_, cnsteps_, alt_ids_;
  DevBuf<float> cprobs_, alt_probs_, logit_tap_;
  std::vector<long> tap_row0_;
  int tap_C_ = 0;
  bool srv_ctc_ = false;
};

struct ClsConfig {
  std::string model_dir, precision = "fp32";
  int device = 0, batch_num = 8;
  double thresh = 0.98;
};

class ClsStage {
 public:
  ~ClsStage();
  bool create(const ClsConfig& cfg, std::string& err, int& code);
  int run(const ocr_img* imgs, int n, int* labels, float* scores, double times[3], std::string& err);
  int run_lines(const std::vector<LineSrc>& lines, int* labels, float* scores, std::string& err);
  hipStream_t stream() const { return stream_; }
  Net& net() { return net_; }
  std::vector<float> tap_probs;

 private:
  ClsConfig cfg_;
  Net net_;
  hipStream_t stream_ = nullptr;
  StageTimer timer_;
  DevBuf<float> lut_, x_, pmax_, probs_;
  DevBuf<int> amax_;
  DevBuf<uint8_t> staging_;
  DevBuf<LineDesc> descs_;
};

bool upload_lines(const ocr_img* imgs, int n, DevBuf<uint8_t>& staging, std::vector<LineSrc>& out, hipStream_t s,
                  std::string& err);

std::vector<float> make_norm_lut(const float mean[3], const float scale[3]);
enum class NormStage { Det, Rec, Cls };
std::vector<float> stage_norm_lut(NormStage st);

}
```

### cpp-paddle-ocr_amd/csrc/stages.hip

```cpp
#include "stages.h"

#include <algorithm>
#include <array>
#include <cmath>
#include <cstring>
#include <fstream>
#include <map>

#include "capi_common.h"

namespace ocr {

#define ST_HIP(expr)                                                              \
  do {                                                                            \
    hipError_t _e = (expr);                                                       \
    if (_e != hipSuccess) {                                                       \
      err = std::string(#expr) + ": " + hipGetErrorString(_e);                    \
      return OCR_ERR_DEVICE;                                                      \
    }                                                                             \
  } while (0)

bool StageTimer::init(std::string& err) {
  for (int i = 0; i < 4; ++i)
    if (hipEventCreate(&ev[i]) != hipSuccess) { err = "hipEventCreate failed"; return false; }
// ... 102 lines not shown
  if (g_stream_create(&stream_) != hipSuccess) { err = "hipStreamCreate failed"; return false; }
  if (!timer_.init(err)) return false;
  const auto lut = stage_norm_lut(NormStage::Det);
  if (!lut_.ensure(lut.size(), err)) return false;
  if (g_memcpy(lut_.p, lut.data(), lut.size() * sizeof(float), hipMemcpyHostToDevice) != hipSuccess) { err = "lut upload failed"; return false; }
  ithresh_ = (int)std::floor(cfg.thresh * 255);
  code = OCR_OK;
  return true;
}

bool DetStage::ensure_post(int count, size_t px, int H, int W, int cap, std::string& err) {
  const int max_cand = 1000;
  pool_cap_ = std::max(1 << 16, (H * W) / 2);
  mask_words_ = mask_words(H, W);
  return labels_.ensure(px, err) && touch_.ensure(px, err) && chunk_cnt_.ensure((size_t)count * 128, err) && ncont_all_.ensure(count, err) && ncont_.ensure(count, err) &&
         starts_.ensure((size_t)count * max_cand, err) && npts_.ensure((size_t)count * max_cand, err) &&
         poff_.ensure((size_t)count * max_cand, err) && pool_.ensure((size_t)count * pool_cap_, err) &&
         iscratch_.ensure((size_t)count * pool_cap_ * 4, err) && cand_boxes_.ensure((size_t)count * max_cand * 8, err) &&
         cand_valid_.ensure((size_t)count * max_cand, err) && status_.ensure(1, err) && pool_need_.ensure(count, err) &&
         out_boxes_.ensure((size_t)count * cap * 8, err) && out_n_.ensure(count, err) &&
         (cfg_.use_dilation ? bitmap2_.ensure(px, err) : true) &&
         (tap_armed_ ? stage_rec_.ensure((size_t)count * max_cand * POST_REC_FLOATS, err) : true) &&
         (cfg_.score_mode == "slow" ? (mask_pool_.ensure((size_t)count * mask_words_, err) && mask_top_.ensure(count, err)) : true);
}

int DetStage::post_launch(PostArgs a, int count, int32_t* boxes, int cap, int* n, std::string& err) {
  a.labels = labels_.p; a.touch = touch_.p; a.chunk_cnt = chunk_cnt_.p; a.ncont_all = ncont_all_.p; a.ncont = ncont_.p;
  a.starts = starts_.p; a.npts = npts_.p; a.poff = poff_.p; a.cand_boxes = cand_boxes_.p; a.cand_valid = cand_valid_.p;
  a.status = status_.p; a.pool_need = pool_need_.p; a.max_cand = 1000;
  a.box_thresh = (float)cfg_.box_thresh; a.unclip_ratio = (float)cfg_.unclip_ratio;
  a.slow = cfg_.score_mode == "slow";
  a.fill_shifted = cfg_.cv_compat != OCR_CV_45;
  a.probe_stop = 0;
#ifdef OCR_DEV_PROBES
  { static const char* stop = getenv("OCR_POST_STOP"); a.probe_stop = stop ? atoi(stop) : 0; }
#endif
  tap_valid_ = false;
  int status = 0;
  auto fill_rec = [&]() -> int {
    if (a.stage_rec) ST_HIP(hipMemsetAsync(a.stage_rec, 0xFF, (size_t)count * a.max_cand * POST_REC_FLOATS * sizeof(float), stream_));
    return OCR_OK;
  };
  auto fetch = [&]() -> int {
    ST_HIP(hipMemcpyAsync(n, out_n_.p, count * sizeof(int), hipMemcpyDeviceToHost, stream_));
    ST_HIP(hipMemcpyAsync(boxes, out_boxes_.p, (size_t)count * cap * 8 * sizeof(int), hipMemcpyDeviceToHost, stream_));
    ST_HIP(hipMemcpyAsync(&status, status_.p, sizeof(int), hipMemcpyDeviceToHost, stream_));
    return OCR_OK;
  };
  for (int attempt = 0;; ++attempt) {
    a.pool = pool_.p; a.iscratch = iscratch_.p; a.pool_cap = pool_cap_;
    if (a.slow) {
      a.mask_pool = mask_pool_.p; a.mask_pool_top = mask_top_.p; a.mask_pool_words = (unsigned)mask_words_;
      ST_HIP(hipMemsetAsync(mask_top_.p, 0, count * sizeof(unsigned), stream_));
    }
    ST_HIP(hipMemsetAsync(status_.p, 0, sizeof(int), stream_));
    if (int rc = fill_rec()) return rc;
    launch_post(a, count, out_boxes_.p, cap, out_n_.p, stream_);
    ST_HIP(hipGetLastError());
    if (int rc = fetch()) return rc;
    if (attempt == 0) timer_.mark(3, stream_);
    ST_HIP(g_stream_sync(stream_));
    if (status && !(status & ~(POST_ERR_HULL | POST_ERR_UNCLIP))) {
      ST_HIP(hipMemsetAsync(status_.p, 0, sizeof(int), stream_));
      if (a.slow) ST_HIP(hipMemsetAsync(mask_top_.p, 0, count * sizeof(unsigned), stream_));
      if (int rc = fill_rec()) return rc;
      launch_post_large(a, count, out_boxes_.p, cap, out_n_.p, stream_);
      ST_HIP(hipGetLastError());
      if (int rc = fetch()) return rc;
      ST_HIP(g_stream_sync(stream_));
    }
    if (!(status & POST_ERR_POOL) || attempt == 4) break;
    std::vector<int> need(count);
    std::vector<unsigned> mneed(a.slow ? count : 0);
    ST_HIP(hipMemcpyAsync(need.data(), pool_need_.p, count * sizeof(int), hipMemcpyDeviceToHost, stream_));
    if (a.slow) ST_HIP(hipMemcpyAsync(mneed.data(), mask_top_.p, count * sizeof(unsigned), hipMemcpyDeviceToHost, stream_));
    ST_HIP(g_stream_sync(stream_));
    const long want_keys = *std::max_element(need.begin(), need.end());
    const size_t want_words = a.slow ? (size_t)*std::max_element(mneed.begin(), mneed.end()) : 0;
    bool grew = false;
    if (want_keys > pool_cap_) {
      if (want_keys > (1L << 28)) break;
      pool_cap_ = (int)((want_keys + 65535) & ~65535L);
      if (!pool_.ensure((size_t)count * pool_cap_, err) || !iscratch_.ensure((size_t)count * pool_cap_ * 4, err)) return OCR_ERR_DEVICE;
      grew = true;
    }
    if (want_words > mask_words_) {
      if (want_words >= (1ul << 31)) break;
      mask_words_ = (want_words + 65535) & ~(size_t)65535;
      if (!mask_pool_.ensure((size_t)count * mask_words_, err)) return OCR_ERR_DEVICE;
      grew = true;
    }
    if (!grew) break;
  }
  if (status) {
    err = "det post-processing scratch exhausted (status " + std::to_string(status) + ")";
    return OCR_ERR_CAPACITY;
  }
  for (int i = 0; i < count; ++i)
    if (n[i] > cap) { err = "more boxes than the caller's capacity"; return OCR_ERR_CAPACITY; }
  return OCR_OK;
}

int DetStage::run_post(int count, int H, int W, const float* prob, float ratio_h, float ratio_w, int src_h, int src_w,
                       int32_t* boxes, int cap, int* n, std::string& err, const uint8_t* bitmap) {
  if (!ensure_post(count, (size_t)count * H * W, H, W, cap, err)) return OCR_ERR_DEVICE;
  const uint8_t* bm = bitmap ? bitmap : bitmap_.p;
  if (cfg_.use_dilation) {
    launch_dilate2(bm, bitmap2_.p, count, H, W, stream_);
    bm = bitmap2_.p;
  }
  PostArgs a{};
  a.bitmap = bm; a.pred = prob;
  a.H = H; a.W = W;
  a.ratio_h = ratio_h; a.ratio_w = ratio_w; a.src_h = src_h; a.src_w = src_w;
  a.stage_rec = tap_armed_ ? stage_rec_.p : nullptr;
  return post_launch(a, count, boxes, cap, n, err);
}

int DetStage::run(const ocr_img* imgs, int count, int32_t* boxes, int cap, int* n, double times[3], std::string& err) {
  if (!imgs || count < 1 || !boxes || !n || cap < 1) { err = "bad argument"; return OCR_ERR_ARG; }
  const int rows = imgs[0].rows, cols = imgs[0].cols;
  for (int i = 0; i < count; ++i) {
    if (!imgs[i].data || imgs[i].rows <= 0 || imgs[i].cols <= 0) { err = "Empty image data provided"; return OCR_ERR_ARG; }
    if (imgs[i].rows != rows || imgs[i].cols != cols) { err = "ocr_det_run_batch needs images of one size"; return OCR_ERR_ARG; }
  }
  ST_HIP(rt_set_device(cfg_.device));
  const size_t row = (size_t)cols * 3, img_bytes = row * rows;
  if (!src_.ensure(img_bytes * count, err)) return OCR_ERR_DEVICE;
  timer_.mark(0, stream_);
  for (int i = 0; i < count; ++i) {
    const size_t stride = imgs[i].row_stride ? imgs[i].row_stride : row;
    ST_HIP(hipMemcpy2DAsync(src_.p + img_bytes * i, row, imgs[i].data, stride, row, rows, hipMemcpyHostToDevice, stream_));
  }
  src_rows_ = rows;
  src_cols_ = cols;
  return run_device(src_.p, img_bytes, row, rows, cols, count, boxes, cap, n, times, err);
}

int DetStage::run_device(const uint8_t* dev_imgs, size_t img_bytes, size_t stride, int rows, int cols, int count,
                         int32_t* boxes, int cap, int* n, double times[3], std::string& err, const float* prob_override) {
  ST_HIP(rt_set_device(cfg_.device));
  int rh, rw;
  float ratio_h, ratio_w;
  resize_shape(rows, cols, cfg_.limit_type, cfg_.limit_side_len, rh, rw, ratio_h, ratio_w);
  const size_t px = (size_t)count * rh * rw;
  const uint8_t* old_bm = bitmap_.p;
  if (!x_.ensure(px * 3, err) || !resized_.ensure(px * 3, err) || !bitmap_.ensure(px, err)) return OCR_ERR_DEVICE;
  if (dev_imgs != src_.p) timer_.mark(0, stream_);
  DetPreArgs pa{};
  pa.src = dev_imgs; pa.src_image_bytes = img_bytes; pa.src_stride = stride;
  pa.N = count; pa.sh = rows; pa.sw = cols; pa.dh = rh; pa.dw = rw; pa.lut = lut_.p; pa.out = x_.p; pa.resized = resized_.p;
  launch_det_pre(pa, stream_);
  timer_.mark(1, stream_);
  if (srv_) {
    if (!srv_->run(x_.p, count, rh, rw, stream_, err)) return OCR_ERR_DEVICE;
    if (!prob_override) launch_bitmap(prob_dev(), bitmap_.p, (long)px, ithresh_, stream_);
  } else {
    if (bitmap_.p != old_bm || bm_n_ == 0) { net_.set_det_bitmap(bitmap_.p, ithresh_); bm_n_ = 1; }
    if (!net_.run(x_.p, count, rh, rw, stream_, err)) return OCR_ERR_DEVICE;
  }
  timer_.mark(2, stream_);
  last_count = count; last_h = rh; last_w = rw;
  const float* pred = prob_dev();
  if (prob_override) {
    launch_bitmap(prob_override, bitmap_.p, (long)px, ithresh_, stream_);
    pred = prob_override;
  }
  src_rows_ = rows;
  src_cols_ = cols;
  const int rc = run_post(count, rh, rw, pred, ratio_h, ratio_w, rows, cols, boxes, cap, n, err);
  net_.collect_timings();
  if (srv_) srv_->collect_timings();
  timer_.read(times);
  return rc;
}

int DetStage::mixed_net(const uint8_t* base, const MixedGroup* groups, int ngroups, const float* prob_override, std::string& err) {
  ST_HIP(rt_set_device(cfg_.device));
  if (srv_) { err = "the server detector runs batches of one image size (a ragged batch of mixed sizes is not built for it)"; return OCR_ERR_ARG; }
  if (!mixed_done_) ST_HIP(hipEventCreateWithFlags(&mixed_done_, hipEventDisableTiming));
  mixed_pix_.assign(ngroups + 1, 0);
  std::vector<int> hs, ws;
  std::vector<std::array<int, 2>> shape(ngroups);
  for (int gi = 0; gi < ngroups; ++gi) {
    float a, b;
    resize_shape(groups[gi].rows, groups[gi].cols, cfg_.limit_type, cfg_.limit_side_len, shape[gi][0], shape[gi][1], a, b);
    mixed_pix_[gi + 1] = mixed_pix_[gi] + (size_t)groups[gi].count * shape[gi][0] * shape[gi][1];
    for (int k = 0; k < groups[gi].count; ++k) { hs.push_back(shape[gi][0]); ws.push_back(shape[gi][1]); }
  }
  const size_t px = mixed_pix_[ngroups];
  const uint8_t* old_bm = bitmap_.p;
  if (!x_.ensure(px * 3, err) || !resized_.ensure(px * 3, err) || !bitmap_.ensure(px, err)) return OCR_ERR_DEVICE;
  timer_.mark(0, stream_);
  for (int gi = 0; gi < ngroups; ++gi) {
    const MixedGroup& g = groups[gi];
    DetPreArgs pa{};
    pa.src = base + g.off; pa.src_image_bytes = (size_t)g.rows * g.cols * 3; pa.src_stride = (size_t)g.cols * 3;
    pa.N = g.count; pa.sh = g.rows; pa.sw = g.cols; pa.dh = shape[gi][0]; pa.dw = shape[gi][1]; pa.lut = lut_.p;
    pa.out = x_.p + mixed_pix_[gi] * 3; pa.resized = resized_.p + mixed_pix_[gi] * 3;
    launch_det_pre(pa, stream_);
  }
  timer_.mark(1, stream_);
  if (bitmap_.p != old_bm || bm_n_ == 0) { net_.set_det_bitmap(bitmap_.p, ithresh_); bm_n_ = 1; }
  if (!net_.run_ragged_images(x_.p, hs.data(), ws.data(), (int)hs.size(), stream_, err)) return OCR_ERR_DEVICE;
  timer_.mark(2, stream_);
  mixed_probs_.assign(ngroups, nullptr);
  mixed_prob_base_ = prob_override ? prob_override : prob_dev();
  for (int gi = 0; gi < ngroups; ++gi) {
    mixed_probs_[gi] = prob_dev() + mixed_pix_[gi];
    if (prob_override) {
      mixed_probs_[gi] = prob_override + groups[gi].prob_off;
      launch_bitmap(mixed_probs_[gi], bitmap_.p + mixed_pix_[gi], (long)(mixed_pix_[gi + 1] - mixed_pix_[gi]), ithresh_, stream_);
    }
  }
  ST_HIP(hipEventRecord(mixed_done_, stream_));
  last_count = (int)hs.size(); last_h = 0; last_w = 0;
  return OCR_OK;
}

int DetStage::post_mixed(const MixedGroup* groups, int ngroups, int32_t* boxes, int cap, int* n, std::string& err) {
  ST_HIP(rt_set_device(cfg_.device));
  if (cfg_.use_dilation) { err = "post_mixed: not with use_dilation"; return OCR_ERR_ARG; }
  std::vector<PostImg> im;
  int Hm = 0, Wm = 0;
  for (int gi = 0; gi < ngroups; ++gi) {
    int rh, rw;
    float ratio_h, ratio_w;
    resize_shape(groups[gi].rows, groups[gi].cols, cfg_.limit_type, cfg_.limit_side_len, rh, rw, ratio_h, ratio_w);
    Hm = std::max(Hm, rh); Wm = std::max(Wm, rw);
    for (int k = 0; k < groups[gi].count; ++k) {
      PostImg q;
      q.h = rh; q.w = rw;
      const size_t off = mixed_pix_[gi] + (size_t)k * rh * rw;
      const size_t poff = (size_t)(mixed_probs_[gi] - mixed_prob_base_) + (size_t)k * rh * rw;
      if (mixed_probs_[gi] < mixed_prob_base_ || off + (size_t)rh * rw >= (1ul << 31) || poff + (size_t)rh * rw >= (1ul << 31)) {
        err = "post_mixed: maps too large for 32-bit offsets";
        return OCR_ERR_CAPACITY;
      }
      q.off = (int)off;
      q.poff = (int)poff;
      q.src_h = groups[gi].rows; q.src_w = groups[gi].cols; q.ratio_h = ratio_h; q.ratio_w = ratio_w;
      im.push_back(q);
    }
  }
  const int count = (int)im.size();
  if (!ensure_post(count, mixed_pix_[ngroups], Hm, Wm, cap, err) || !post_img_.ensure(count, err)) return OCR_ERR_DEVICE;
  ST_HIP(hipMemcpyAsync(post_img_.p, im.data(), (size_t)count * sizeof(PostImg), hipMemcpyHostToDevice, stream_));
  PostArgs a{};
  a.img = post_img_.p;
  a.bitmap = bitmap_.p; a.pred = mixed_prob_base_;
  a.H = Hm; a.W = Wm;
  return post_launch(a, count, boxes, cap, n, err);
}

int DetStage::post_group(const float* prob, const uint8_t* bitmap, const MixedGroup& g, hipEvent_t wait_for, int32_t* boxes, int cap,
                         int* n, std::string& err) {
  ST_HIP(rt_set_device(cfg_.device));
  if (wait_for) ST_HIP(hipStreamWaitEvent(stream_, wait_for, 0));
  int rh, rw;
  float ratio_h, ratio_w;
  resize_shape(g.rows, g.cols, cfg_.limit_type, cfg_.limit_side_len, rh, rw, ratio_h, ratio_w);
  src_rows_ = g.rows;
  src_cols_ = g.cols;
  return run_post(g.count, rh, rw, prob, ratio_h, ratio_w, g.rows, g.cols, boxes, cap, n, err, bitmap);
}

int DetStage::post_only(const float* prob, int rows, int cols, int src_rows, int src_cols, int32_t* boxes, int cap, int* n,
                        std::string& err) {
  if (!prob || rows <= 0 || cols <= 0 || !boxes || !n || cap < 1) { err = "bad argument"; return OCR_ERR_ARG; }
  ST_HIP(rt_set_device(cfg_.device));
  const size_t px = (size_t)rows * cols;
  if (!prob_in_.ensure(px, err) || !bitmap_.ensure(px, err)) return OCR_ERR_DEVICE;
  bm_n_ = 0;
  ST_HIP(hipMemcpyAsync(prob_in_.p, prob, px * sizeof(float), hipMemcpyHostToDevice, stream_));
  launch_bitmap(prob_in_.p, bitmap_.p, (long)px, ithresh_, stream_);
  last_count = 1; last_h = rows; last_w = cols;
  const float ratio_h = float(rows) / float(src_rows), ratio_w = float(cols) / float(src_cols);
  const int rc = run_post(1, rows, cols, prob_in_.p, ratio_h, ratio_w, src_rows, src_cols, boxes, cap, n, err);
  tap_valid_ = tap_armed_ && rc == OCR_OK;
  tap_h_ = rows; tap_w_ = cols;
  return rc;
}

static_assert(POST_REC_FLOATS == OCR_POST_REC_FLOATS, "the stage record of kernels_post.h is the one include/ocr_hip.h describes");
int DetStage::post_stages(ocr_post_stages* o, std::string& err) {
  if (!o || !o->bitmap || !o->starts || !o->npts || !o->voff || !o->verts || !o->cand_valid || !o->cand_boxes || !o->record) {
    err = "post_stages: null pointer";
    return OCR_ERR_ARG;
  }
  const bool was_valid = tap_valid_;
  tap_armed_ = true;
  if (!was_valid) { err = "post_stages: no recorded ocr_det_post on this handle (the tap is armed from now on)"; return OCR_ERR_ARG; }
  ST_HIP(rt_set_device(cfg_.device));
  const int max_cand = 1000;
  const size_t px = (size_t)tap_h_ * tap_w_;
  if (px >= (1ul << 24)) { err = "post_stages: the record counts mask pixels in a float, maps below 2^24 pixels only"; return OCR_ERR_ARG; }
  int nall = 0, nc = 0;
  ST_HIP(g_memcpy(&nall, ncont_all_.p, sizeof(int), hipMemcpyDeviceToHost));
  ST_HIP(g_memcpy(&nc, ncont_.p, sizeof(int), hipMemcpyDeviceToHost));
  if (nc < 0 || nc > max_cand) { err = "post_stages: border count out of range"; return OCR_ERR_DEVICE; }
  std::vector<int> npts(nc), poff(nc);
  if (nc) {
    ST_HIP(g_memcpy(npts.data(), npts_.p, (size_t)nc * sizeof(int), hipMemcpyDeviceToHost));
    ST_HIP(g_memcpy(poff.data(), poff_.p, (size_t)nc * sizeof(int), hipMemcpyDeviceToHost));
  }
  long nverts = 0, pool_end = 0;
  for (int c = 0; c < nc; ++c) {
    if (npts[c] <= 2 || poff[c] < 0) continue;
    if ((long)poff[c] + npts[c] > pool_cap_) { err = "post_stages: border outside the key pool"; return OCR_ERR_DEVICE; }
    nverts += npts[c];
    pool_end = std::max(pool_end, (long)poff[c] + npts[c]);
  }
  o->rows = tap_h_; o->cols = tap_w_; o->ncont_all = nall; o->ncont = nc; o->nverts = (int)nverts;
  if (px > o->cap_pixels || nc > o->cap_borders || nverts > o->cap_verts) { err = "post_stages: output capacity too small"; return OCR_ERR_CAPACITY; }
  ST_HIP(g_memcpy(o->bitmap, bitmap_dev(), px, hipMemcpyDeviceToHost));
  if (nc) {
    ST_HIP(g_memcpy(o->starts, starts_.p, (size_t)nc * sizeof(int), hipMemcpyDeviceToHost));
    memcpy(o->npts, npts.data(), (size_t)nc * sizeof(int));
    ST_HIP(g_memcpy(o->cand_valid, cand_valid_.p, (size_t)nc * sizeof(int), hipMemcpyDeviceToHost));
    ST_HIP(g_memcpy(o->cand_boxes, cand_boxes_.p, (size_t)nc * 8 * sizeof(int), hipMemcpyDeviceToHost));
    ST_HIP(g_memcpy(o->record, stage_rec_.p, (size_t)nc * POST_REC_FLOATS * sizeof(float), hipMemcpyDeviceToHost));
  }
  std::vector<unsigned long long> keys((size_t)pool_end);
  if (pool_end) ST_HIP(g_memcpy(keys.data(), pool_.p, (size_t)pool_end * sizeof(unsigned long long), hipMemcpyDeviceToHost));
  long k = 0;
  for (int c = 0; c < nc; ++c) {
    if (npts[c] <= 2 || poff[c] < 0) { o->voff[c] = -1; continue; }
    o->voff[c] = (int)k;
    for (int i = 0; i < npts[c]; ++i, ++k) {
      const unsigned long long key = keys[(size_t)poff[c] + i];
      o->verts[2 * k] = (int)(key >> 48) - 16384;
      o->verts[2 * k + 1] = (int)((key >> 32) & 0xffff) - 16384;
    }
  }
  return OCR_OK;
}

RecStage::~RecStage() {
  if (stream_) (void)hipStreamDestroy(stream_);
}

bool RecStage::create(const RecConfig& cfg, std::string& err, int& code) {
  cfg_ = cfg;
  code = OCR_ERR_ARG;
  if (cfg.precision != "fp32" && cfg.precision != "fp16") { err = "precision '" + cfg.precision + "' is not implemented (fp32 | fp16)"; return false; }
  if (cfg.batch_num < 1 || cfg.img_h < 1 || cfg.img_w < 1) { err = "bad rec shape"; return false; }
  if (cfg.sort_mode != OCR_SORT_STD && cfg.sort_mode != OCR_SORT_STABLE && cfg.sort_mode != OCR_SORT_MSVC_STRICT) { err = "unknown sort_mode"; return false; }
  code = ocr_rt_init(cfg.device);
  if (code) { err = ocr_last_error(); return false; }
  code = OCR_ERR_MODEL;
  std::ifstream in(cfg.label_path);
  if (!in) { err = "no such label file: " + cfg.label_path; return false; }
  labels_.clear();
  labels_.push_back("#");
  for (std::string line; std::getline(in, line);) labels_.push_back(line);
  labels_.push_back(" ");
  WeightMap w;
// ... 175 lines not shown
  if (T > 0 && T > rec_plan::uniform_step_cap(tensor_w)) { err = "rec step buffer too small"; return OCR_ERR_CAPACITY; }
  return OCR_OK;
}

int RecStage::LinesCtx::mobile_logits(const Slot& sl, View& v) {
  if (topk <= 0) return OCR_OK;
  Net::HeadLogits hl;
  if (!st.net_.head_logits(hl, err)) return OCR_ERR_DEVICE;
  if (hl.C != C) { err = "dictionary size does not match the CTC head"; return OCR_ERR_MODEL; }
  if (sl.ragged)
    for (int j = 0; j < sl.count; ++j)
      if ((int)hl.row0.size() != sl.count + 1 || hl.row0[j] != d[sl.first + j].step0) { err = "ragged logits rows do not match the step table"; return OCR_ERR_DEVICE; }
  v.logits = hl.ptr;
  v.pitch = hl.pitch;
  return OCR_OK;
}

int RecStage::LinesCtx::run_srv(Slot& sl, View& v) {
  SrvNet& srv = *st.srv_;
  const int Wt = items[sl.first].tensor_w;
  launch_line_pre(st.descs_.p + sl.first, sl.count, imgH, Wt, st.lut_.p, false, st.x_.p, st.stream_);
  if (!srv.run(st.x_.p, sl.count, imgH, Wt, st.stream_, err)) return OCR_ERR_DEVICE;
  const SrvTensor& ot = srv.tensor(srv.output_tid());
  if (const int rc = check_output(ot.h, ot.c, ot.w, Wt)) return rc;
  sl.T = ot.w;
  const float* out = (const float*)srv.tensor_ptr(srv.output_tid());
  if (srv.ctc_partials())
    srv::launch_ctc_reduce(out, (long)sl.count * sl.T, srv.ctc_slots(), srv.ctc_step(), st.amax_.p + sl.step_off, st.pmax_.p + sl.step_off,
                           st.stream_);
  else
    srv::launch_argmax_softmax(out, (long)sl.count * sl.T, ot.c, ot.cs, st.amax_.p + sl.step_off, st.pmax_.p + sl.step_off, srv.half(),
                               st.stream_);
  v.T = sl.T;
  v.logits = out;
  v.pitch = ot.cs;
  return OCR_OK;
}

int RecStage::LinesCtx::run_ragged(Slot& sl, View& v) {
  st.net_.set_head_outputs(nullptr, st.amax_.p + sl.step_off, st.pmax_.p + sl.step_off);
  widths.resize(sl.count);
  long pix = 0;
  for (int j = 0; j < sl.count; ++j) { widths[j] = items[sl.first + j].tensor_w; pix += (long)imgH * widths[j]; }
  launch_line_pre_ragged(st.descs_.p + sl.first, sl.count, pix, imgH, st.lut_.p, st.x_.p, st.stream_);
  if (!st.net_.run_ragged(st.x_.p, imgH, widths.data(), sl.count, st.stream_, err)) return OCR_ERR_DEVICE;
  v.lines_dev = st.descs_.p + sl.first;
  return mobile_logits(sl, v);
}

int RecStage::LinesCtx::run_uniform(Slot& sl, View& v) {
  st.net_.set_head_outputs(nullptr, st.amax_.p + sl.step_off, st.pmax_.p + sl.step_off);
  const int Wt = items[sl.first].tensor_w;
  launch_line_pre(st.descs_.p + sl.first, sl.count, imgH, Wt, st.lut_.p, false, st.x_.p, st.stream_);
  if (!st.net_.run(st.x_.p, sl.count, imgH, Wt, st.stream_, err)) return OCR_ERR_DEVICE;
  const TensorDesc& ot = st.net_.tensor(st.net_.output_tid());
  if (const int rc = check_output(ot.h, ot.c, ot.w, Wt)) return rc;
  v.T = sl.T = ot.w;
  return mobile_logits(sl, v);
}

int RecStage::LinesCtx::decode(const Slot& sl, const View& v) {
  const int* amax = st.amax_.p + sl.step_off;
  const float* pmax = st.pmax_.p + sl.step_off;
  const size_t o = (size_t)sl.first * max_len;
  if (!co) {
    if (v.lines_dev) launch_ctc_ragged(amax, pmax, v.lines_dev, sl.count, max_len, st.ids_.p + o, st.lens_.p + sl.first, st.scores_.p + sl.first, st.stream_);
    else launch_ctc(amax, pmax, sl.count, v.T, max_len, st.ids_.p + o, st.lens_.p + sl.first, st.scores_.p + sl.first, st.stream_);
    return OCR_OK;
  }
  launch_ctc_chars(amax, pmax, v.lines_dev, sl.count, v.T, max_len, st.ids_.p + o, st.lens_.p + sl.first, st.scores_.p + sl.first,
                   st.csteps_.p + o, st.cnsteps_.p + o, st.cprobs_.p + o, st.stream_);
  if (topk <= 0) return OCR_OK;
  launch_ctc_topk(v.logits, v.pitch, C, topk, v.lines_dev, sl.count, v.T, max_len, st.lens_.p + sl.first, st.csteps_.p + o, st.cprobs_.p + o,
                  st.alt_ids_.p + o * topk, st.alt_probs_.p + o * topk, st.stream_);
  if (tap_logits) {
    const LineDesc& last = d[sl.first + sl.count - 1];
    const size_t rows = v.lines_dev ? (size_t)(last.step0 + last.steps) : (size_t)sl.count * v.T;
    ST_HIP(hipMemcpy2DAsync(st.logit_tap_.p + sl.step_off * (size_t)C, (size_t)C * sizeof(float), v.logits, (size_t)v.pitch * sizeof(float),
                            (size_t)C * sizeof(float), rows, hipMemcpyDeviceToDevice, st.stream_));
  }
  return OCR_OK;
}

int RecStage::LinesCtx::read_back() {
  const size_t ni = items.size();
  bool ok = fetch(h_ids, st.ids_.p, ni * max_len);
  ok = ok && fetch(h_lens, st.lens_.p, ni);
  ok = ok && fetch(h_scores, st.scores_.p, ni);
  if (st.want_taps) {
    ok = ok && fetch(h_amax, st.amax_.p, step_total);
    ok = ok && fetch(h_pmax, st.pmax_.p, step_total);
  }
  if (co) {
    ok = ok && fetch(h_steps, st.csteps_.p, nchar);
    ok = ok && fetch(h_nsteps, st.cnsteps_.p, nchar);
    ok = ok && fetch(h_cprobs, st.cprobs_.p, nchar);
  }
  if (topk > 0) {
    ok = ok && fetch(h_alt_ids, st.alt_ids_.p, nchar * topk);
    ok = ok && fetch(h_alt_probs, st.alt_probs_.p, nchar * topk);
  }
  return ok ? OCR_OK : OCR_ERR_DEVICE;
}

int RecStage::LinesCtx::scatter(int32_t* ids, int* lens, float* scores) {
  for (const Slot& sl : slots)
    for (int j = 0; j < sl.count; ++j) {
      const int q = sl.first + j, li = items[q].line;
      if (h_lens[q] > max_len) { err = "text longer than max_len"; return OCR_ERR_CAPACITY; }
      lens[li] = h_lens[q];
      scores[li] = h_scores[q];
      memcpy(ids + (size_t)li * max_len, h_ids.data() + (size_t)q * max_len, (size_t)h_lens[q] * sizeof(int));
      const int T = sl.ragged ? d[q].steps : sl.T;
      const size_t step = step_of(sl, j);
      if (co) {
        const size_t from = (size_t)q * max_len, to = (size_t)li * max_len, len = (size_t)h_lens[q];
        if (co->steps) memcpy(co->steps + to, h_steps.data() + from, len * sizeof(int));
        if (co->nsteps) memcpy(co->nsteps + to, h_nsteps.data() + from, len * sizeof(int));
        if (co->probs) memcpy(co->probs + to, h_cprobs.data() + from, len * sizeof(float));
        if (co->geom) { co->geom[3 * li] = T; co->geom[3 * li + 1] = items[q].tensor_w; co->geom[3 * li + 2] = items[q].resize_w; }
        if (topk > 0) {
          memcpy(co->alt_ids + to * topk, h_alt_ids.data() + from * topk, len * topk * sizeof(int));
          memcpy(co->alt_probs + to * topk, h_alt_probs.data() + from * topk, len * topk * sizeof(float));
        }
        if (tap_logits) st.tap_row0_[li] = (long)step;
      }
      st.tap_T[li] = T;
      if (st.want_taps) {
        st.tap_off[li] = (int)st.tap_amax.size();
        st.tap_amax.insert(st.tap_amax.end(), h_amax.begin() + step, h_amax.begin() + step + T);
        st.tap_pmax.insert(st.tap_pmax.end(), h_pmax.begin() + step, h_pmax.begin() + step + T);
      }
    }
  return OCR_OK;
}

int RecStage::run_lines(const std::vector<LineSrc>& lines, const std::vector<int>& seg, int32_t* ids, int max_len,
                        int* lens, float* scores, std::string& err, const CharOut* co) {
  const int n = (int)lines.size();
  const int topk = co ? co->topk : 0;
  if (srv_) srv_->set_ctc_partials(topk > 0 ? false : srv_ctc_);
  else net_.set_keep_logits(topk > 0);
  tap_row0_.assign(n, -1);
  LinesCtx c(*this, lines, co, max_len, err);
  int rc = c.plan(seg);
  if (rc) return rc;
  tap_T.assign(n, 0);
  tap_off.assign(n, 0);
  tap_amax.clear();
  tap_pmax.clear();
  for (int i = 0; i < n; ++i) { lens[i] = 0; scores[i] = 0.f; }
  if (c.items.empty()) return OCR_OK;
  if ((rc = c.describe())) return rc;
  for (LinesCtx::Slot& sl : c.slots) {
    LinesCtx::View v;
    rc = srv_ ? c.run_srv(sl, v) : sl.ragged ? c.run_ragged(sl, v) : c.run_uniform(sl, v);
    if (!rc) rc = c.decode(sl, v);
    if (rc) return rc;
  }
  if ((rc = c.read_back())) return rc;
  ST_HIP(g_stream_sync(stream_));
  net_.collect_timings();
  if (srv_) srv_->collect_timings();
  return c.scatter(ids, lens, scores);
}

ClsStage::~ClsStage() {
  if (stream_) (void)hipStreamDestroy(stream_);
}

bool ClsStage::create(const ClsConfig& cfg, std::string& err, int& code) {
  cfg_ = cfg;
  code = OCR_ERR_ARG;
  if (cfg.precision != "fp32" && cfg.precision != "fp16") { err = "precision '" + cfg.precision + "' is not implemented (fp32 | fp16)"; return false; }
  if (cfg.batch_num < 1) { err = "cls_batch_num must be >= 1"; return false; }
  code = ocr_rt_init(cfg.device);
  if (code) { err = ocr_last_error(); return false; }
  code = OCR_ERR_MODEL;
  WeightMap w;
  if (!load_model_dir(cfg.model_dir, nullptr, "cls", w, err)) return false;
  if (!net_.load(embedded_plan("cls"), w, err, cfg.precision == "fp16")) return false;
  code = OCR_ERR_DEVICE;
  if (g_stream_create(&stream_) != hipSuccess) { err = "hipStreamCreate failed"; return false; }
  if (!timer_.init(err)) return false;
  const auto lut = stage_norm_lut(NormStage::Cls);
  if (!lut_.ensure(lut.size(), err)) return false;
  if (g_memcpy(lut_.p, lut.data(), lut.size() * sizeof(float), hipMemcpyHostToDevice) != hipSuccess) { err = "lut upload failed"; return false; }
  code = OCR_OK;
  return true;
}

int ClsStage::run(const ocr_img* imgs, int n, int* labels, float* scores, double times[3], std::string& err) {
  if (n < 0 || (n > 0 && (!imgs || !labels || !scores))) { err = "bad argument"; return OCR_ERR_ARG; }
  if (times) times[0] = times[1] = times[2] = 0;
  if (n == 0) return OCR_OK;
  ST_HIP(rt_set_device(cfg_.device));
  timer_.mark(0, stream_);
  std::vector<LineSrc> lines;
  if (!upload_lines(imgs, n, staging_, lines, stream_, err)) return OCR_ERR_DEVICE;
  timer_.mark(1, stream_);
  const int rc = run_lines(lines, labels, scores, err);
  timer_.mark(2, stream_);
  timer_.mark(3, stream_);
  (void)g_stream_sync(stream_);
  timer_.read(times);
  return rc;
}

int ClsStage::run_lines(const std::vector<LineSrc>& lines, int* labels, float* scores, std::string& err) {
  const int n = (int)lines.size();
  const int imgH = 48, imgW = 192;
  std::vector<LineDesc> d(n);
  for (int i = 0; i < n; ++i) {
    const LineSrc& L = lines[i];
    d[i] = LineDesc::make(L.img, L.stride, L.x, L.y, L.w, L.h, rec_plan::rec_resize_w(L.w, L.h, imgH, imgW), i, imgH);
  }
  if (!descs_.ensure(n, err) || !x_.ensure((size_t)n * imgH * imgW * 3, err)) return OCR_ERR_DEVICE;
  ST_HIP(hipMemcpyAsync(descs_.p, d.data(), n * sizeof(LineDesc), hipMemcpyHostToDevice, stream_));
  launch_line_pre(descs_.p, n, imgH, imgW, lut_.p, true, x_.p, stream_);
  const int* old_a = amax_.p;
  const float* old_p = pmax_.p;
  const float* old_q = probs_.p;
  if (!amax_.ensure(n, err) || !pmax_.ensure(n, err) || !probs_.ensure((size_t)n * 2, err)) return OCR_ERR_DEVICE;
  if (amax_.p != old_a || pmax_.p != old_p || probs_.p != old_q || !old_a) net_.set_head_outputs(probs_.p, amax_.p, pmax_.p);
  if (!net_.run(x_.p, n, imgH, imgW, stream_, err)) return OCR_ERR_DEVICE;
  tap_probs.resize((size_t)n * 2);
  ST_HIP(hipMemcpyAsync(labels, amax_.p, n * sizeof(int), hipMemcpyDeviceToHost, stream_));
  ST_HIP(hipMemcpyAsync(scores, pmax_.p, n * sizeof(float), hipMemcpyDeviceToHost, stream_));
  ST_HIP(hipMemcpyAsync(tap_probs.data(), probs_.p, tap_probs.size() * sizeof(float), hipMemcpyDeviceToHost, stream_));
  ST_HIP(g_stream_sync(stream_));
  net_.collect_timings();
  return OCR_OK;
}

}
```

### include/ocr_hip.h

```cpp
#ifndef OCR_HIP_H_
#define OCR_HIP_H_

#include <stddef.h>
#include <stdint.h>

#ifdef __cplusplus
extern "C" {
#endif

#define OCR_OK 0
#define OCR_ERR_ARG (-1)
#define OCR_ERR_MODEL (-2)
#define OCR_ERR_DEVICE (-3)
#define OCR_ERR_CAPACITY (-4)

const char* ocr_last_error(void);
int ocr_rt_init(int device_id);
int ocr_rt_device_count(void);
int ocr_rt_set_wait_mode(int mode);
int ocr_rt_get_wait_mode(void);

typedef struct ocr_img {
  const uint8_t* data;
  int rows, cols;
// ... 180 lines not shown
  OCR_RAW_BIT1_INV
} ocr_raw_kind;
typedef struct ocr_raw_frame {
  int width, height;
  int kind;
  int bottom_up;
  size_t row_stride;
  uint8_t palette[1024];
  const uint8_t* data;
  size_t data_len;
} ocr_raw_frame;
int ocr_raw_decode(const ocr_raw_frame* frame, int device_id, uint8_t* bgr, size_t cap_bytes);
int ocr_raw_time(const ocr_raw_frame* frame, int device_id, int iters, double ms[2]);
int ocr_raw_time_batch(const ocr_raw_frame* const* frames, int count, int device_id, int iters, double ms[2]);
int ocr_pipe_stage_frames(ocr_pipe* h, int slot, const ocr_jpeg_frame* const* jpegs, const ocr_png_frame* const* pngs,
                          const ocr_raw_frame* const* raws, int count);
typedef struct ocr_tiff_frame {
  int width, height;
  int photometric;
  int bits_per_sample;
  int samples_per_pixel;
  int planar;
  int predictor;
  int big_endian;
  int premultiply;
  int tile_width, tile_height;
  uint8_t palette[1024];
  const uint8_t* data;
  size_t data_len;
} ocr_tiff_frame;
int ocr_tiff_decode(const ocr_tiff_frame* frame, int device_id, uint8_t* bgr, size_t cap_bytes);
int ocr_tiff_time(const ocr_tiff_frame* frame, int device_id, int iters, double ms[2]);
int ocr_tiff_time_batch(const ocr_tiff_frame* const* frames, int count, int device_id, int iters, double ms[2]);
typedef struct ocr_tiff_chunk {
  uint64_t byte_off;
  uint32_t byte_len;
  uint32_t rows;
} ocr_tiff_chunk;
typedef struct ocr_tiff_coded {
  ocr_tiff_frame frame;
  int compression;
  const ocr_tiff_chunk* chunks;
  size_t chunks_len;
  const uint8_t* bytes;
  size_t bytes_len;
} ocr_tiff_coded;
int ocr_tiff_expand(const ocr_tiff_coded* coded, int device_id, uint8_t* out, size_t cap);
int ocr_tiff_decode_coded(const ocr_tiff_coded* coded, int device_id, uint8_t* bgr, size_t cap_bytes);
int ocr_tiff_time_coded(const ocr_tiff_coded* coded, int device_id, int iters, double ms[3]);
int ocr_tiff_time_coded_batch(const ocr_tiff_coded* const* coded, int count, int device_id, int iters, double ms[3]);
int ocr_tiff_inflate(const ocr_tiff_coded* coded, int device_id, uint8_t* out, size_t cap, uint32_t* produced);
int ocr_tiff_decode_deflate(const ocr_tiff_coded* coded, int device_id, uint8_t* bgr, size_t cap_bytes);
int ocr_tiff_time_deflate(const ocr_tiff_coded* coded, int device_id, int iters, double ms[3]);
int ocr_tiff_time_deflate_batch(const ocr_tiff_coded* const* coded, int count, int device_id, int iters, double ms[3]);
typedef struct ocr_webp_transform {
  int kind;
  int bits;
  const uint32_t* data;
  size_t data_len;
} ocr_webp_transform;
typedef struct ocr_webp_frame {
  int width, height;
  const uint32_t* argb;
  size_t argb_len;
  int ntransforms;
  ocr_webp_transform transforms[4];
} ocr_webp_frame;
int ocr_webp_decode(const ocr_webp_frame* frame, int device_id, uint8_t* bgr, size_t cap_bytes);
int ocr_webp_time(const ocr_webp_frame* frame, int device_id, int iters, double ms[2]);
int ocr_webp_time_batch(const ocr_webp_frame* const* frames, int count, int device_id, int iters, double ms[2]);
typedef struct ocr_vp8_mb {
  uint8_t modes[16];
  uint8_t is_i4x4;
  uint8_t uvmode;
  uint8_t level;
  uint8_t ilevel;
  uint8_t hev;
  uint8_t inner;
  uint8_t segment, skip;
  uint32_t nz_y;
  uint32_t nz_uv;
  uint32_t present;
  uint32_t coeff_off;
} ocr_vp8_mb;
typedef struct ocr_vp8_frame {
  int width, height;
  int filter_type;
  const ocr_vp8_mb* mbs;
  size_t mbs_len;
  const int16_t* coeffs;
  size_t coeffs_len;
} ocr_vp8_frame;
int ocr_vp8_decode(const ocr_vp8_frame* frame, int device_id, uint8_t* bgr, size_t cap_bytes);
int ocr_vp8_time(const ocr_vp8_frame* frame, int device_id, int iters, double ms[2]);
int ocr_vp8_time_batch(const ocr_vp8_frame* const* frames, int count, int device_id, int iters, double ms[2]);
typedef struct ocr_j2k_tilecomp {
  int x0, y0, x1, y1;
  int levels;
  int comp;
  uint32_t step_off;
  uint32_t reserved;
  uint64_t coeff_off;
} ocr_j2k_tilecomp;
typedef struct ocr_j2k_frame {
  int width, height;
  int x0, y0;
  int ncomp;
  int prec;
  int transform;
  int mct;
  int chan[3];
  const ocr_j2k_tilecomp* tcs;
  size_t tcs_len;
  const float* steps;
  size_t steps_len;
  const int32_t* coeffs;
  size_t coeffs_len;
} ocr_j2k_frame;
int ocr_j2k_decode(const ocr_j2k_frame* frame, int device_id, uint8_t* bgr, size_t cap_bytes);
int ocr_j2k_time(const ocr_j2k_frame* frame, int device_id, int iters, double ms[2]);
int ocr_j2k_time_batch(const ocr_j2k_frame* const* frames, int count, int device_id, int iters, double ms[2]);
typedef struct ocr_j2k_cblk {
  uint32_t tc;
  uint32_t at;
  uint64_t byte_off;
  uint32_t byte_len;
  uint16_t w, h;
  uint8_t orient;
  uint8_t numbps;
  uint8_t passes;
  uint8_t reserved;
  uint32_t reserved2;
} ocr_j2k_cblk;
typedef struct ocr_j2k_coded {
  ocr_j2k_frame frame;
  const ocr_j2k_cblk* cblks;
  size_t cblks_len;
  const uint8_t* bytes;
  size_t bytes_len;
} ocr_j2k_coded;
int ocr_j2k_tier1(const ocr_j2k_coded* coded, int device_id, int32_t* coeffs, size_t cap);
int ocr_j2k_decode_coded(const ocr_j2k_coded* coded, int device_id, uint8_t* bgr, size_t cap_bytes);
int ocr_j2k_time_coded(const ocr_j2k_coded* coded, int device_id, int iters, double ms[3]);
int ocr_j2k_time_coded_batch(const ocr_j2k_coded* const* coded, int count, int device_id, int iters, double ms[3]);
typedef enum ocr_frame_kind { OCR_FRAME_JPEG = 0, OCR_FRAME_PNG = 1, OCR_FRAME_RAW = 2, OCR_FRAME_TIFF = 3, OCR_FRAME_WEBP = 4, OCR_FRAME_VP8 = 5, OCR_FRAME_J2K = 6, OCR_FRAME_J2K_CODED = 7, OCR_FRAME_TIFF_CODED = 8, OCR_FRAME_TIFF_DEFLATE = 9 } ocr_frame_kind;
typedef struct ocr_coded_frame {
  int kind;
  const void* frame;
} ocr_coded_frame;
int ocr_pipe_stage_batch(ocr_pipe* h, int slot, const ocr_coded_frame* frames, int count);
const char* ocr_pipe_label(ocr_pipe* h, int id);
int ocr_pipe_det_shape(ocr_pipe* h, int rows, int cols, int* net_rows, int* net_cols);
int ocr_pipe_stats(ocr_pipe* h, long long out[3]);
int ocr_pipe_timing(ocr_pipe* h, int enable);
int ocr_pipe_timing_filter(ocr_pipe* h, const char* substr);
int ocr_pipe_timing_report(ocr_pipe* h, char* buf, size_t cap);

int ocr_rotate_crop(const uint8_t* bgr, int rows, int cols, size_t row_stride, const int32_t* boxes, int n, uint8_t* out,
                    size_t out_cap, size_t* out_off, int* out_rows, int* out_cols);
int ocr_rotate_crop_shape(int rows, int cols, const int32_t* box, int* out_rows, int* out_cols);

int ocr_rotate180_rois(uint8_t* bgr, int rows, int cols, size_t row_stride, const int32_t* rects, int n);

int ocr_dev_alloc(void** p, size_t bytes);
int ocr_dev_free(void* p);
int ocr_dev_upload(void* dst, const void* src, size_t bytes);
int ocr_dev_download(void* dst, const void* src, size_t bytes);
int ocr_dev_sync(void);
int ocr_dev_copy_time(void* dst, const void* src, size_t bytes, int iters, double* ms);

typedef struct ocr_net ocr_net;
int ocr_net_create(const char* kind, const char* model_dir, const char* weights, int device_id, ocr_net** out);
int ocr_net_create_precision(const char* kind, const char* model_dir, const char* weights, int device_id, const char* precision,
                             ocr_net** out);
void ocr_net_destroy(ocr_net* h);
int ocr_net_forward(ocr_net* h, const float* x, int N, int H, int W, int keep_all);
int ocr_net_forward_ragged(ocr_net* h, const float* x, int N, int H, const int* widths, int keep_all);
int ocr_net_forward_ragged_images(ocr_net* h, const float* x, int N, const int* heights, const int* widths, int keep_all);
int ocr_net_num_tensors(ocr_net* h);
int ocr_net_tensor_exists(ocr_net* h, int tid);
int ocr_net_fetch(ocr_net* h, int tid, float* out, size_t cap_floats, int dims[4]);
int ocr_net_timing(ocr_net* h, int enable);
int ocr_net_timing_report(ocr_net* h, char* buf, size_t cap);

typedef struct ocr_srv_net ocr_srv_net;
int ocr_srv_net_create(const char* kind, const char* model_dir, int device_id, const char* precision, ocr_srv_net** out);
void ocr_srv_net_destroy(ocr_srv_net* h);
int ocr_srv_net_forward(ocr_srv_net* h, const float* x, int N, int H, int W, int keep_all);
int ocr_srv_net_rerun(ocr_srv_net* h, int N, int H, int W, int iters);
int ocr_srv_net_num_tensors(ocr_srv_net* h);
int ocr_srv_net_fetch(ocr_srv_net* h, int tid, float* out, size_t cap_floats, int dims[4]);
int ocr_srv_net_set_ctc(ocr_srv_net* h, int on);
int ocr_srv_net_ctc_tail(ocr_srv_net* h, int32_t* amax, float* pmax, long cap_rows, long* rows, int* slots, int* step);
int ocr_srv_net_timing(ocr_srv_net* h, int enable);
int ocr_srv_net_timing_report(ocr_srv_net* h, char* buf, size_t cap);
int ocr_srv_net_num_launches(ocr_srv_net* h);
int ocr_srv_net_launch_info(ocr_srv_net* h, int i, char* name, size_t name_cap, int* out_tid, int* in_tids, int in_cap, int* n_in);
int ocr_srv_net_run_launches(ocr_srv_net* h, int first, int count);
int ocr_srv_net_upload(ocr_srv_net* h, int tid, const float* data, size_t count);
int ocr_srv_net_create_plan(const char* plan_text, const char* params_path, int device_id, const char* precision, ocr_srv_net** out);
int ocr_srv_net_set_config(ocr_srv_net* h, int cfg, int strict);
int ocr_srv_gemm_num_configs(void);
const char* ocr_srv_gemm_config_name(int cfg);
int ocr_srv_gemm_config_bn(int cfg);

int ocr_selftest_refuse_launch(const char* substr);
int ocr_selftest_lds_memo(void);

int ocr_selftest_unclip(const int32_t* quads, const double* deltas, int n, int64_t* out, int cap, int* counts, double* trig);
int ocr_selftest_unclip_box(const float* boxes, float unclip_ratio, int n, float* out14, int* status);

#define OCR_POST_REC_FLOATS 12
#define OCR_POST_REC_FILL 0xFFFFFFFFu
typedef struct ocr_post_stages {
  size_t cap_pixels;
  int cap_borders;
  int cap_verts;
  uint8_t* bitmap;
  int32_t *starts, *npts, *voff, *verts, *cand_valid, *cand_boxes;
  float* record;
  int rows, cols, ncont_all, ncont, nverts;
} ocr_post_stages;
int ocr_det_post_stages(ocr_det* h, ocr_post_stages* out);

#define OCR_SELFTEST_FILL 0xA5
#define OCR_SELFTEST_GUARD 256
#define OCR_PAD_REC 0
#define OCR_PAD_CLS 1
#define OCR_STAGE_REC 1
#define OCR_STAGE_CLS 2
int ocr_selftest_det_pre(const uint8_t* buf, size_t buf_bytes, size_t src_offset, size_t src_stride, size_t src_image_bytes, int N,
                         int sh, int sw, int dh, int dw, float* out, uint8_t* resized);
int ocr_selftest_line_pre(const uint8_t* img, int rows, int cols, size_t stride, const int32_t* lines, int n, int imgH, int imgW,
                          int nslots, int pad_mode, int stage, float* out);
int ocr_selftest_line_pre_ragged(const uint8_t* img, int rows, int cols, size_t stride, const int32_t* lines, int n, int imgH,
                                 int stage, float* out);

typedef struct ocr_warp_case {
  uint64_t src_off, sstride;
  int32_t sw, sh, dw, dh, rot, bw0;
  double m[9];
} ocr_warp_case;
int ocr_selftest_warp_crops(const uint8_t* src, size_t src_bytes, const ocr_warp_case* cases, int n, int max_pixels,
                            const uint64_t* out_off, size_t out_bytes, uint8_t* out);
int ocr_selftest_rotate180_groups(uint8_t* buf, size_t buf_bytes, const int64_t* rois, int n, const int32_t* seg, int ngroups);
int ocr_selftest_crop_plan(int rows, int cols, const int32_t* box8, int32_t* fields, double* minv);
int ocr_selftest_rotation_groups(const int32_t* rects, const int32_t* views, int n, int32_t* order, int32_t* seg, int* ngroups);

int ocr_selftest_softmax_argmax(const float* logits, long rows, int C, float* probs, int32_t* amax, float* pmax);
int ocr_selftest_head_combine(const float* hmax, const float* hsum, const int32_t* hidx, long rows, int groups, int32_t* amax,
                              float* pmax);
int ocr_selftest_srv_argmax(const float* logits, long rows, int C, int ld, int one_pass, int32_t* amax, float* pmax);
int ocr_selftest_ctc_reduce(const float* part, long rows, int slots, int step, int32_t* amax, float* pmax);
int ocr_selftest_ctc(const int32_t* amax, const float* pmax, long nsteps_total, int nlines, int T, const int32_t* lines, int max_len,
                     int chars, int32_t* ids, int32_t* lens, float* scores, int32_t* steps, int32_t* nsteps, float* probs);
int ocr_selftest_topk_lines(const float* rows, int nlines, int T, int C, int pitch, const int32_t* lens, const int32_t* steps,
                            const float* p0, int max_len, int k, int32_t* out_ids, float* out_probs);

int ocr_selftest_rec_head(const char* model_dir, const char* weights, const char* precision, const float* rows, long nrows, int K,
                          int lines, int imgH, int imgW, int mode, int32_t* amax, float* pmax, float* logits, int* ncols, char* names,
                          size_t names_cap);

int ocr_probe(const float* a, const float* b, float* out, int n);

#ifdef __cplusplus
}
#endif
#endif
```

Baseline: 1229.

## Add pipe planner, persistent chain threads, and optional staggered net gating

Moves the image-to-chain partitioning into a separate pipe_plan module, replaces per-call std::thread creation with a persistent thread pool, and adds an optional DenseGate that serialises network launches across chains in a staggered order using events. Workers are now created lazily as the plan requires. The default stays at two chains in 'together' mode, so the main default-path change is reusing threads instead of spawning them on every call. It also adds event-lifetime cleanup and a stats counter.

```diff
diff --git a/cpp-paddle-ocr_amd/binding.py b/cpp-paddle-ocr_amd/binding.py
--- a/cpp-paddle-ocr_amd/binding.py
+++ b/cpp-paddle-ocr_amd/binding.py
@@ -954,7 +954,7 @@
             "ocr_j2k_tier1", "ocr_j2k_decode_coded", "ocr_j2k_time_coded", "ocr_j2k_time_coded_batch",
             "ocr_tiff_expand", "ocr_tiff_decode_coded", "ocr_tiff_time_coded", "ocr_tiff_time_coded_batch",
             "ocr_tiff_inflate", "ocr_tiff_decode_deflate", "ocr_tiff_time_deflate", "ocr_tiff_time_deflate_batch",
-            "ocr_pipe_label", "ocr_pipe_det_shape", "ocr_pipe_stats", "ocr_pipe_timing", "ocr_pipe_timing_filter", "ocr_pipe_timing_report", "ocr_dev_alloc",
+            "ocr_pipe_label", "ocr_pipe_det_shape", "ocr_pipe_stats", "ocr_pipe_stats_n", "ocr_pipe_timing", "ocr_pipe_timing_filter", "ocr_pipe_timing_report", "ocr_dev_alloc",
             "ocr_dev_free", "ocr_dev_upload", "ocr_dev_download", "ocr_dev_sync", "ocr_dev_copy_time", "ocr_rotate_crop", "ocr_rotate_crop_shape", "ocr_rotate180_rois"]
 
 
diff --git a/cpp-paddle-ocr_amd/csrc/capi_net.hip b/cpp-paddle-ocr_amd/csrc/capi_net.hip
--- a/cpp-paddle-ocr_amd/csrc/capi_net.hip
+++ b/cpp-paddle-ocr_amd/csrc/capi_net.hip
@@ -32,6 +32,7 @@
     o.dwpw_force_upw = (int)num("OCR_DWPW_FORCE_UPW", 0);
     if (const char* e = getenv("OCR_DWPW_T4")) o.dwpw_t4_thin = e[0] == 't';
     o.trace_slice = (int)num("OCR_TRACE_SLICE", 0);
+    if (const char* e = getenv("OCR_PIPE_CHAINS")) o.pipe_chains = e;
   });
   return o;
 }
diff --git a/cpp-paddle-ocr_amd/csrc/hip_guard.h b/cpp-paddle-ocr_amd/csrc/hip_guard.h
--- a/cpp-paddle-ocr_amd/csrc/hip_guard.h
+++ b/cpp-paddle-ocr_amd/csrc/hip_guard.h
@@ -1,6 +1,7 @@
 #pragma once
 #include <hip/hip_runtime.h>
 
+#include <atomic>
 #include <mutex>
 #include <shared_mutex>
 
@@ -38,14 +39,24 @@
 
 int rt_wait_mode();
 void rt_set_wait_mode(int m);
+inline std::atomic<long long> g_wait_events_created{0}, g_wait_events_alive{0};
+struct WaitEvents {
+  hipEvent_t ev[64] = {};
+  ~WaitEvents() {
+    for (hipEvent_t e : ev)
+      if (e) { (void)hipEventDestroy(e); --g_wait_events_alive; }
+  }
+};
 inline hipError_t g_stream_sync(hipStream_t s) {
   if (rt_wait_mode() == 0) return hipStreamSynchronize(s);
-  thread_local hipEvent_t ev[64] = {};
+  thread_local WaitEvents mine;
   const int d = rt_current_device();
-  hipEvent_t& e = ev[d >= 0 && d < 64 ? d : 0];
+  hipEvent_t& e = mine.ev[d >= 0 && d < 64 ? d : 0];
   if (!e) {
     const hipError_t c = hipEventCreateWithFlags(&e, hipEventBlockingSync | hipEventDisableTiming);
     if (c != hipSuccess) { e = nullptr; (void)hipGetLastError(); return hipStreamSynchronize(s); }
+    ++g_wait_events_created;
+    ++g_wait_events_alive;
   }
   const hipError_t r = hipEventRecord(e, s);
   if (r != hipSuccess) return r;
diff --git a/cpp-paddle-ocr_amd/csrc/pipe.hip b/cpp-paddle-ocr_amd/csrc/pipe.hip
--- a/cpp-paddle-ocr_amd/csrc/pipe.hip
+++ b/cpp-paddle-ocr_amd/csrc/pipe.hip
@@ -1,6 +1,7 @@
 #include <algorithm>
 #include <array>
 #include <chrono>
+#include <condition_variable>
 #include <cstring>
 #include <functional>
 #include <map>
@@ -10,7 +11,9 @@
 #include "capi_common.h"
 #include "crop.h"
 #include "frame_kinds.h"
+#include "pipe_plan.h"
 #include "rot_groups.h"
+#include "rt_options.h"
 #include "stages.h"
 
 using namespace ocr;
@@ -65,6 +68,58 @@
   if (hipGetLastError() != hipSuccess) { err = "rotation launch failed"; return OCR_ERR_DEVICE; }
   return OCR_OK;
 }
+
+struct DenseGate {
+  static constexpr int kRing = 8, kMaxChains = 4;
+  std::mutex m;
+  std::condition_variable cv;
+  hipEvent_t ring[kRing] = {};
+  hipEvent_t last = nullptr;
+  int next = 0;
+  bool busy = false;
+  bool started[kMaxChains] = {true, true, true, true};
+  int start_after[kMaxChains] = {-1, -1, -1, -1};
+  ~DenseGate() { for (hipEvent_t e : ring) if (e) (void)hipEventDestroy(e); }
+  bool init() {
+    for (hipEvent_t& e : ring)
+      if (!e && hipEventCreateWithFlags(&e, hipEventDisableTiming) != hipSuccess) { e = nullptr; (void)hipGetLastError(); return false; }
+    return true;
+  }
+  void begin_call(const std::vector<int>& after) {
+    std::lock_guard<std::mutex> lk(m);
+    for (int c = 0; c < kMaxChains; ++c) {
+      start_after[c] = c < (int)after.size() ? after[c] : -1;
+      started[c] = c >= (int)after.size();
+    }
+  }
+  void enter(int chain, hipStream_t s) {
+    std::unique_lock<std::mutex> lk(m);
+    const int before = started[chain] ? -1 : start_after[chain];
+    cv.wait(lk, [&] { return !busy && (before < 0 || started[before]); });
+    busy = true;
+    if (last) (void)hipStreamWaitEvent(s, last, 0);
+  }
+  void leave(int chain, hipStream_t s) {
+    std::lock_guard<std::mutex> lk(m);
+    hipEvent_t e = ring[next];
+    next = (next + 1) % kRing;
+    if (e && hipEventRecord(e, s) == hipSuccess) last = e;
+    busy = false;
+    started[chain] = true;
+    cv.notify_all();
+  }
+  void finish(int chain) {
+    std::lock_guard<std::mutex> lk(m);
+    started[chain] = true;
+    cv.notify_all();
+  }
+};
+struct ChainGate : NetGate {
+  DenseGate* all = nullptr;
+  int chain = 0;
+  void enter(hipStream_t s) override { all->enter(chain, s); }
+  void leave(hipStream_t s) override { all->leave(chain, s); }
+};
 
 struct PipeWorker {
   DetStage det;
@@ -107,8 +162,14 @@
     if (!d->create(det_cfg, err, code)) return code ? code : OCR_ERR_DEVICE;
     d->net().set_timing_filter(timing_filter);
     d->net().enable_timing(timing_on);
+    d->gate = det.gate;
     det_extra.push_back(std::move(d));
     return OCR_OK;
+  }
+  void set_gate(NetGate* g) {
+    det.gate = g;
+    for (auto& d : det_extra) d->gate = g;
+    rec.gate = g;
   }
 
   int run_images(uint8_t* base, const std::vector<StageSlot::Img>& imgs, const std::vector<StageSlot::Group>& groups, const float* probs,
@@ -355,18 +416,93 @@
   }
 };
 
+struct ChainThreads {
+  std::vector<std::thread> th;
+  std::mutex m;
+  std::condition_variable cv_job, cv_done;
+  const std::function<void(int)>* job = nullptr;
+  unsigned long gen = 0;
+  int njobs = 0, pending = 0, device = 0;
+  bool stop = false;
+  long long created = 0;
+  ~ChainThreads() {
+    { std::lock_guard<std::mutex> lk(m); stop = true; }
+    cv_job.notify_all();
+    for (auto& t : th) t.join();
+  }
+  void loop(int id) {
+    (void)rt_set_device(device);
+    unsigned long seen = 0;
+    std::unique_lock<std::mutex> lk(m);
+    for (;;) {
+      cv_job.wait(lk, [&] { return stop || gen != seen; });
+      if (stop) return;
+      seen = gen;
+      if (id > njobs) continue;
+      const std::function<void(int)>* f = job;
+      lk.unlock();
+      (*f)(id);
+      lk.lock();
+      if (--pending == 0) cv_done.notify_one();
+    }
+  }
+  void run(int n, const std::function<void(int)>& fn) {
+    {
+      std::lock_guard<std::mutex> lk(m);
+      while ((int)th.size() < n - 1) {
+        const int id = (int)th.size() + 1;
+        th.emplace_back([this, id] { loop(id); });
+        ++created;
+      }
+      job = &fn;
+      njobs = pending = n - 1;
+      ++gen;
+    }
+    cv_job.notify_all();
+    fn(0);
+    std::unique_lock<std::mutex> lk(m);
+    cv_done.wait(lk, [&] { return pending == 0; });
+    job = nullptr;
+  }
+};
+
 struct ocr_pipe {
   PipeWorker w0;
   std::vector<std::unique_ptr<PipeWorker>> extra;
-  int phases = 2;
-  int parts_per_chain = 1;
+  int phases = 0;
+  int chains = 2, parts_per_chain = 1;
+  pipe_plan::Mode mode = pipe_plan::kTogether;
+  DenseGate gate;
+  ChainGate chain_gate[DenseGate::kMaxChains];
+  bool gate_ok = false;
+  DetConfig det_cfg;
+  RecConfig rec_cfg;
+  ClsConfig cls_cfg;
+  bool has_cls = false;
+  int crop_mode = OCR_CROP_BOUNDING_RECT;
   int device = 0;
+  int add_worker(std::string& err) {
+    std::unique_ptr<PipeWorker> w(new PipeWorker());
+    const int rc = w->create(det_cfg, rec_cfg, has_cls ? &cls_cfg : nullptr, crop_mode, err);
+    if (rc) return rc;
+    w->det_lanes = w0.det_lanes;
+    w->det_ragged = w0.det_ragged;
+    w->det_post_ragged = w0.det_post_ragged;
+    w->timing_on = w0.timing_on;
+    w->timing_filter = w0.timing_filter;
+    for (Net* net : {&w->det.net(), w->cls ? &w->cls->net() : nullptr, &w->rec.net()})
+      if (net) { net->set_timing_filter(w0.timing_filter); net->enable_timing(w0.timing_on); }
+    extra.push_back(std::move(w));
+    return OCR_OK;
+  }
   StageSlot slots[2];
   hipStream_t copy_stream = nullptr;
   FrameScratch frame_scratch;
   DevBuf<uint8_t> work;
   DevBuf<uint8_t> work_chain[4];
   PipeWorker* worker(int c) { return c == 0 ? &w0 : (c >= 1 && c <= (int)extra.size() ? extra[c - 1].get() : nullptr); }
+
+  ChainThreads threads;
 
   ~ocr_pipe() { if (copy_stream) (void)hipStreamDestroy(copy_stream); }
 
@@ -471,41 +607,31 @@
                  std::vector<std::vector<ocr_word>>& out_words, std::vector<std::vector<int32_t>>& out_ids, double times[3], std::string& err,
                  CharLists* out_chars = nullptr) {
     const int count = (int)imgs.size();
-    const int nchains = (int)std::min<size_t>(1 + extra.size(), (size_t)count);
-    if (nchains < 2) return w0.run_images(base, imgs, groups, probs, out_words, out_ids, times, err, out_chars);
-    const int K = (int)std::min<size_t>((size_t)nchains * parts_per_chain, (size_t)count);
+    std::vector<pipe_plan::Group> sizes;
+    for (const auto& g : groups) sizes.push_back(pipe_plan::Group{g.rows, g.cols, g.count});
+    const pipe_plan::Plan P = pipe_plan::make(count, sizes, chains, chains * parts_per_chain, mode);
+    if (P.chains < 2) return w0.run_images(base, imgs, groups, probs, out_words, out_ids, times, err, out_chars);
+    while ((int)extra.size() + 1 < P.chains) {
+      const int rc = add_worker(err);
+      if (rc) return rc;
+    }
+    const int nchains = P.chains, K = (int)P.parts.size();
     std::vector<std::vector<StageSlot::Img>> pi(K);
     std::vector<std::vector<StageSlot::Group>> pg(K);
     std::vector<std::vector<int>> gidx(K);
-    std::vector<size_t> load(K, 0);
-    auto give = [&](int p, const StageSlot::Group& g, int first, int n) {
-      int rh = 0, rw = 0;
-      { float a, b; DetStage::resize_shape(g.rows, g.cols, w0.det.cfg().limit_type, w0.det.cfg().limit_side_len, rh, rw, a, b); }
-      StageSlot::Group ng = g;
-      ng.first = (int)pi[p].size();
-      ng.count = n;
-      ng.off = g.off + (size_t)first * g.rows * g.cols * 3;
-      ng.prob_off = g.prob_off + (size_t)first * rh * rw;
-      pg[p].push_back(ng);
-      for (int k = 0; k < n; ++k) { pi[p].push_back(imgs[g.first + first + k]); gidx[p].push_back(g.first + first + k); }
-      load[p] += (size_t)n * g.rows * g.cols;
-    };
-    size_t total = 0;
-    for (const auto& g : groups) total += (size_t)g.count * g.rows * g.cols;
-    const size_t share = (total + K - 1) / K;
-    for (const auto& g : groups) {
-      const size_t px = (size_t)g.rows * g.cols;
-      int first = 0;
-      while (first < g.count) {
-        const int p = (int)(std::min_element(load.begin(), load.end()) - load.begin());
-        const int left = g.count - first;
-        const size_t room = share > load[p] ? share - load[p] : 0;
-        int n = left;
-        if ((size_t)left * px > room + px / 2) n = (int)std::min<size_t>(left, std::max<size_t>(1, (room + px / 2) / px));
-        give(p, g, first, n);
-        first += n;
-      }
-    }
+    for (int p = 0; p < K; ++p)
+      for (const pipe_plan::Range& r : P.parts[p].ranges) {
+        const StageSlot::Group& g = groups[r.group];
+        int rh = 0, rw = 0;
+        { float a, b; DetStage::resize_shape(g.rows, g.cols, w0.det.cfg().limit_type, w0.det.cfg().limit_side_len, rh, rw, a, b); }
+        StageSlot::Group ng = g;
+        ng.first = (int)pi[p].size();
+        ng.count = r.count;
+        ng.off = g.off + (size_t)r.first * g.rows * g.cols * 3;
+        ng.prob_off = g.prob_off + (size_t)r.first * rh * rw;
+        pg[p].push_back(ng);
+        for (int k = 0; k < r.count; ++k) { pi[p].push_back(imgs[r.image + k]); gidx[p].push_back(r.image + k); }
+      }
     if (g_stream_sync(w0.det.stream()) != hipSuccess) { err = "det stream sync failed"; return OCR_ERR_DEVICE; }
     std::vector<std::vector<std::vector<ocr_word>>> W(K);
     std::vector<std::vector<std::vector<int32_t>>> I(K);
@@ -513,18 +639,20 @@
     std::vector<std::array<double, 3>> t(K, std::array<double, 3>{0, 0, 0});
     std::vector<int> rc(K, OCR_OK);
     std::vector<std::string> errs(K);
-    auto chain = [&](int c) {
-      PipeWorker& w = c == 0 ? w0 : *extra[c - 1];
-      for (int p = c; p < K; p += nchains) {
-        if (pi[p].empty()) continue;
+    const bool staggered = mode == pipe_plan::kStaggered && gate_ok;
+    if (staggered) gate.begin_call(P.start_after);
+    for (int c = 0; c < nchains; ++c) worker(c)->set_gate(staggered ? &chain_gate[c] : nullptr);
+    const std::function<void(int)> chain = [&](int c) {
+      PipeWorker& w = *worker(c);
+      for (int p = P.first[c]; p < K; p += nchains) {
         rc[p] = w.run_images(base, pi[p], pg[p], probs, W[p], I[p], t[p].data(), errs[p], out_chars ? &Ch[p] : nullptr);
-        if (rc[p]) return;
-      }
+        if (rc[p]) break;
+      }
+      if (staggered) gate.finish(c);
     };
-    std::vector<std::thread> th;
-    for (int c = 1; c < nchains; ++c) th.emplace_back([&, c]() { (void)rt_set_device(device); chain(c); });
-    chain(0);
-    for (auto& x : th) x.join();
+    threads.device = device;
+    threads.run(nchains, chain);
+    for (int c = 0; c < nchains; ++c) worker(c)->set_gate(nullptr);
     for (int p = 0; p < K; ++p)
       if (rc[p]) { err = errs[p]; return rc[p]; }
     out_words.assign(count, {});
@@ -616,8 +744,23 @@
   h->device = c->det.device_id;
   if (c->crop_mode != OCR_CROP_BOUNDING_RECT && c->crop_mode != OCR_CROP_ROTATE) return fail(OCR_ERR_ARG, "unknown crop_mode");
   if (c->phases < 0 || c->phases > 4) return fail(OCR_ERR_ARG, "phases must be 0 (default) or 1..4");
-  h->phases = c->phases ? c->phases : 2;
+  h->phases = c->phases;
   if (const char* e = getenv("OCR_PIPE_PHASES")) h->phases = std::min(4, std::max(1, atoi(e)));
+  if (h->phases) {
+    h->chains = h->phases;
+  } else {
+    h->chains = pipe_plan::kDefaultChains;
+    h->mode = pipe_plan::kDefaultMode;
+    const std::string& o = rt_options().pipe_chains;
+    if (!o.empty() && o[0] >= '1' && o[0] <= '4') {
+      h->chains = o[0] - '0';
+      h->mode = pipe_plan::kStaggered;
+      size_t k = 1;
+      if (k + 1 < o.size() + 0 && o[k] == 'x' && o[k + 1] >= '1' && o[k + 1] <= '4') { h->parts_per_chain = o[k + 1] - '0'; k += 2; }
+      if (k < o.size() && o[k] == 't') h->mode = pipe_plan::kTogether;
+    }
+  }
+  for (int c = 0; c < DenseGate::kMaxChains; ++c) { h->chain_gate[c].all = &h->gate; h->chain_gate[c].chain = c; }
   std::string err;
   DetConfig d;
   d.model_dir = c->det.model_dir; d.device = c->det.device_id;
@@ -643,19 +786,19 @@
   if (const char* e = getenv("OCR_DET_LANES")) lanes = std::min(32, std::max(1, atoi(e)));
   int rc = h->w0.create(d, r, c->enable_cls ? &k : nullptr, c->crop_mode, err);
   if (rc) return fail(rc, err);
-  h->w0.det_lanes = lanes;
-  for (int p = 1; p < h->phases; ++p) {
-    h->extra.emplace_back(new PipeWorker());
-    rc = h->extra.back()->create(d, r, c->enable_cls ? &k : nullptr, c->crop_mode, err);
-    if (rc) return fail(rc, err);
-  }
-  h->w0.det_lanes = std::max(1, (lanes + h->phases - 1) / h->phases);
-  for (auto& w : h->extra) w->det_lanes = h->w0.det_lanes;
+  h->w0.det_lanes = std::max(1, (lanes + h->chains - 1) / h->chains);
   if (const char* e = getenv("OCR_DET_RAGGED")) {
     h->w0.det_ragged = e[0] != '0';
     h->w0.det_post_ragged = e[0] != 'n';
-    for (auto& w : h->extra) { w->det_ragged = h->w0.det_ragged; w->det_post_ragged = h->w0.det_post_ragged; }
-  }
+  }
+  h->det_cfg = d; h->rec_cfg = r; h->cls_cfg = k; h->has_cls = c->enable_cls != 0; h->crop_mode = c->crop_mode;
+  const int eager = h->phases ? h->phases : std::min(h->chains, 2);
+  for (int p = 1; p < eager; ++p) {
+    rc = h->add_worker(err);
+    if (rc) return fail(rc, err);
+  }
+  CAPI_HIP(rt_set_device(h->device));
+  h->gate_ok = h->mode == pipe_plan::kStaggered && h->gate.init();
   priority_anchor(h->device, 2);
   *out = h.release();
   return OCR_OK;
@@ -878,10 +1021,10 @@
   for (auto& w : h->extra) w->timing_on = enable != 0;
   return OCR_OK;
 }
-int ocr_pipe_stats(ocr_pipe* h, long long out[3]) {
-  if (!h || !out) return fail(OCR_ERR_ARG, "null argument");
-  out[0] = out[1] = out[2] = 0;
-  auto add = [&](Net& n) { out[0] += n.stats().runs; out[1] += n.stats().binds; out[2] += n.stats().graph_replays; };
+int ocr_pipe_stats_n(ocr_pipe* h, long long* out, int n) {
+  if (!h || !out || n < 3) return fail(OCR_ERR_ARG, "null argument");
+  for (int k = 0; k < n; ++k) out[k] = 0;
+  auto add = [&](Net& net) { out[0] += net.stats().runs; out[1] += net.stats().binds; out[2] += net.stats().graph_replays; };
   std::vector<PipeWorker*> ws{&h->w0};
   for (auto& w : h->extra) ws.push_back(w.get());
   for (PipeWorker* w : ws) {
@@ -890,8 +1033,13 @@
     if (w->cls) add(w->cls->net());
     add(w->rec.net());
   }
+  if (n > 3) out[3] = g_wait_events_created.load();
+  if (n > 4) out[4] = g_wait_events_alive.load();
+  if (n > 5) { std::lock_guard<std::mutex> lk(h->threads.m); out[5] = h->threads.created; }
+  if (n > 6) out[6] = 1 + (long long)h->extra.size();
   return OCR_OK;
 }
+int ocr_pipe_stats(ocr_pipe* h, long long out[3]) { return ocr_pipe_stats_n(h, out, 3); }
 int ocr_pipe_timing_filter(ocr_pipe* h, const char* substr) {
   if (!h) return fail(OCR_ERR_ARG, "null handle");
   const std::string f = substr ? substr : "";
diff --git a/cpp-paddle-ocr_amd/csrc/pipe_plan.h b/cpp-paddle-ocr_amd/csrc/pipe_plan.h
--- /dev/null
+++ b/cpp-paddle-ocr_amd/csrc/pipe_plan.h
@@ -0,0 +1,73 @@
+#pragma once
+#include <algorithm>
+#include <cstddef>
+#include <vector>
+
+namespace ocr {
+namespace pipe_plan {
+
+struct Group { int rows, cols, count; };
+struct Range { int group, first, count, image; };
+struct Part {
+  int chain = 0;
+  int order = 0;
+  std::vector<Range> ranges;
+  int images() const { int n = 0; for (const Range& r : ranges) n += r.count; return n; }
+};
+struct Plan {
+  int chains = 0;
+  std::vector<Part> parts;
+  std::vector<int> first;
+  std::vector<int> start_after;
+};
+
+enum Mode { kTogether = 0, kStaggered = 1 };
+
+inline Plan make(int count, const std::vector<Group>& groups, int chains, int parts, Mode mode) {
+  Plan P;
+  if (count < 1 || chains < 1) return P;
+  const int nchains = std::min(chains, count);
+  const int K = std::min(std::max(parts, nchains), count);
+  std::vector<Part> deal(K);
+  std::vector<size_t> load(K, 0);
+  size_t total = 0;
+  for (const Group& g : groups) total += (size_t)g.count * g.rows * g.cols;
+  const size_t share = (total + K - 1) / K;
+  int image = 0;
+  for (int gi = 0; gi < (int)groups.size(); ++gi) {
+    const Group& g = groups[gi];
+    const size_t px = (size_t)g.rows * g.cols;
+    int first = 0;
+    while (first < g.count) {
+      const int p = (int)(std::min_element(load.begin(), load.end()) - load.begin());
+      const int left = g.count - first;
+      const size_t room = share > load[p] ? share - load[p] : 0;
+      int n = left;
+      if ((size_t)left * px > room + px / 2) n = (int)std::min<size_t>(left, std::max<size_t>(1, (room + px / 2) / px));
+      deal[p].ranges.push_back(Range{gi, first, n, image + first});
+      load[p] += (size_t)n * px;
+      first += n;
+    }
+    image += g.count;
+  }
+  for (Part& part : deal)
+    if (!part.ranges.empty()) P.parts.push_back(std::move(part));
+  const int np = (int)P.parts.size();
+  P.chains = std::min(nchains, np);
+  P.first.assign(P.chains, -1);
+  for (int p = 0; p < np; ++p) {
+    P.parts[p].chain = p % P.chains;
+    P.parts[p].order = p / P.chains;
+    if (P.parts[p].order == 0) P.first[P.parts[p].chain] = p;
+  }
+  P.start_after.assign(P.chains, -1);
+  if (mode == kStaggered)
+    for (int c = 1; c < P.chains; ++c) P.start_after[c] = c - 1;
+  return P;
+}
+
+constexpr int kDefaultChains = 2;
+constexpr Mode kDefaultMode = kTogether;
+
+}
+}
diff --git a/cpp-paddle-ocr_amd/csrc/rt_options.h b/cpp-paddle-ocr_amd/csrc/rt_options.h
--- a/cpp-paddle-ocr_amd/csrc/rt_options.h
+++ b/cpp-paddle-ocr_amd/csrc/rt_options.h
@@ -19,6 +19,7 @@
   int dwpw_force_upw = 0;
   bool dwpw_t4_thin = false;
   int trace_slice = 0;
+  std::string pipe_chains;
 };
 const RtOptions& rt_options();
 
diff --git a/cpp-paddle-ocr_amd/csrc/stages.h b/cpp-paddle-ocr_amd/csrc/stages.h
--- a/cpp-paddle-ocr_amd/csrc/stages.h
+++ b/cpp-paddle-ocr_amd/csrc/stages.h
@@ -36,6 +36,20 @@
   ~StageTimer();
   void mark(int i, hipStream_t s) { (void)hipEventRecord(ev[i], s); }
   void read(double times[3]);
+};
+
+struct NetGate {
+  virtual ~NetGate() {}
+  virtual void enter(hipStream_t s) = 0;
+  virtual void leave(hipStream_t s) = 0;
+};
+struct NetGateScope {
+  NetGate* g;
+  hipStream_t s;
+  NetGateScope(NetGate* gate, hipStream_t stream) : g(gate), s(stream) { if (g) g->enter(s); }
+  ~NetGateScope() { if (g) g->leave(s); }
+  NetGateScope(const NetGateScope&) = delete;
+  NetGateScope& operator=(const NetGateScope&) = delete;
 };
 
 struct DetConfig {
@@ -70,6 +84,7 @@
   hipStream_t stream() const { return stream_; }
   Net& net() { return net_; }
   int last_count = 0, last_h = 0, last_w = 0;
+  NetGate* gate = nullptr;
   const float* prob_dev() const { return srv_ ? (const float*)srv_->tensor_ptr(srv_->output_tid()) : net_.tensor_ptr(net_.output_tid()); }
   SrvNet* srv() { return srv_.get(); }
   const uint8_t* bitmap_dev() const { return cfg_.use_dilation ? bitmap2_.p : bitmap_.p; }
@@ -151,6 +166,7 @@
   static constexpr int kSrvLinesPerLaunch = 1024;
   static_assert((unsigned long long)kSrvLinesPerLaunch * (12 * 80 * 768) * sizeof(float) < 0xfffffff0ull, "a server launch passes the buffer-descriptor guard");
   int max_lines_per_launch = 4096;
+  NetGate* gate = nullptr;
   const std::vector<std::string>& labels() const { return labels_; }
   hipStream_t stream() const { return stream_; }
   Net& net() { return net_; }
diff --git a/cpp-paddle-ocr_amd/csrc/stages.hip b/cpp-paddle-ocr_amd/csrc/stages.hip
--- a/cpp-paddle-ocr_amd/csrc/stages.hip
+++ b/cpp-paddle-ocr_amd/csrc/stages.hip
@@ -278,12 +278,15 @@
   pa.N = count; pa.sh = rows; pa.sw = cols; pa.dh = rh; pa.dw = rw; pa.lut = lut_.p; pa.out = x_.p; pa.resized = resized_.p;
   launch_det_pre(pa, stream_);
   timer_.mark(1, stream_);
-  if (srv_) {
-    if (!srv_->run(x_.p, count, rh, rw, stream_, err)) return OCR_ERR_DEVICE;
-    if (!prob_override) launch_bitmap(prob_dev(), bitmap_.p, (long)px, ithresh_, stream_);
-  } else {
-    if (bitmap_.p != old_bm || bm_n_ == 0) { net_.set_det_bitmap(bitmap_.p, ithresh_); bm_n_ = 1; }
-    if (!net_.run(x_.p, count, rh, rw, stream_, err)) return OCR_ERR_DEVICE;
+  {
+    NetGateScope in_turn(gate, stream_);
+    if (srv_) {
+      if (!srv_->run(x_.p, count, rh, rw, stream_, err)) return OCR_ERR_DEVICE;
+      if (!prob_override) launch_bitmap(prob_dev(), bitmap_.p, (long)px, ithresh_, stream_);
+    } else {
+      if (bitmap_.p != old_bm || bm_n_ == 0) { net_.set_det_bitmap(bitmap_.p, ithresh_); bm_n_ = 1; }
+      if (!net_.run(x_.p, count, rh, rw, stream_, err)) return OCR_ERR_DEVICE;
+    }
   }
   timer_.mark(2, stream_);
   last_count = count; last_h = rh; last_w = rw;
@@ -328,7 +331,10 @@
   }
   timer_.mark(1, stream_);
   if (bitmap_.p != old_bm || bm_n_ == 0) { net_.set_det_bitmap(bitmap_.p, ithresh_); bm_n_ = 1; }
-  if (!net_.run_ragged_images(x_.p, hs.data(), ws.data(), (int)hs.size(), stream_, err)) return OCR_ERR_DEVICE;
+  {
+    NetGateScope in_turn(gate, stream_);
+    if (!net_.run_ragged_images(x_.p, hs.data(), ws.data(), (int)hs.size(), stream_, err)) return OCR_ERR_DEVICE;
+  }
   timer_.mark(2, stream_);
   mixed_probs_.assign(ngroups, nullptr);
   mixed_prob_base_ = prob_override ? prob_override : prob_dev();
@@ -810,11 +816,14 @@
   for (int i = 0; i < n; ++i) { lens[i] = 0; scores[i] = 0.f; }
   if (c.items.empty()) return OCR_OK;
   if ((rc = c.describe())) return rc;
-  for (LinesCtx::Slot& sl : c.slots) {
-    LinesCtx::View v;
-    rc = srv_ ? c.run_srv(sl, v) : sl.ragged ? c.run_ragged(sl, v) : c.run_uniform(sl, v);
-    if (!rc) rc = c.decode(sl, v);
-    if (rc) return rc;
+  {
+    NetGateScope in_turn(gate, stream_);
+    for (LinesCtx::Slot& sl : c.slots) {
+      LinesCtx::View v;
+      rc = srv_ ? c.run_srv(sl, v) : sl.ragged ? c.run_ragged(sl, v) : c.run_uniform(sl, v);
+      if (!rc) rc = c.decode(sl, v);
+      if (rc) return rc;
+    }
   }
   if ((rc = c.read_back())) return rc;
   ST_HIP(g_stream_sync(stream_));
diff --git a/cpp-paddle-ocr_amd/host/pipe_plan_check.cpp b/cpp-paddle-ocr_amd/host/pipe_plan_check.cpp
--- /dev/null
+++ b/cpp-paddle-ocr_amd/host/pipe_plan_check.cpp
@@ -0,0 +1,48 @@
+#include <cstdio>
+#include <vector>
+
+#include "../csrc/pipe_plan.h"
+
+using namespace ocr;
+
+static bool read_ints(FILE* f, int* out, int n) {
+  for (int i = 0; i < n; ++i)
+    if (fscanf(f, "%d", out + i) != 1) return false;
+  return true;
+}
+
+int main(int argc, char** argv) {
+  if (argc != 2 || argv[1][0] == '-') {
+    fprintf(stderr, "usage: pipe_plan_check <cases>\n");
+    return 2;
+  }
+  FILE* f = fopen(argv[1], "r");
+  if (!f) { fprintf(stderr, "cannot read %s\n", argv[1]); return 2; }
+  int head[5];
+  for (int k = 0; read_ints(f, head, 5); ++k) {
+    const int count = head[0], chains = head[1], parts = head[2], mode = head[3], ngroups = head[4];
+    if (count < 0 || chains < 1 || chains > 64 || parts < 1 || parts > 4096 || (mode != 0 && mode != 1) || ngroups < 0 || ngroups > (1 << 16)) return 2;
+    std::vector<pipe_plan::Group> groups(ngroups);
+    long sum = 0;
+    for (pipe_plan::Group& g : groups) {
+      if (!read_ints(f, &g.rows, 1) || !read_ints(f, &g.cols, 1) || !read_ints(f, &g.count, 1)) return 2;
+      if (g.rows < 1 || g.cols < 1 || g.count < 1 || g.rows > (1 << 15) || g.cols > (1 << 15) || g.count > (1 << 20)) return 2;
+      sum += g.count;
+    }
+    if (sum != count) return 2;
+    const pipe_plan::Plan P = pipe_plan::make(count, groups, chains, parts, mode ? pipe_plan::kStaggered : pipe_plan::kTogether);
+    printf("case %d\nchains %d\nparts %zu\n", k, P.chains, P.parts.size());
+    for (const pipe_plan::Part& p : P.parts) {
+      printf("part %d %d %zu\n", p.chain, p.order, p.ranges.size());
+      for (const pipe_plan::Range& r : p.ranges) printf("%d %d %d %d\n", r.group, r.first, r.count, r.image);
+    }
+    printf("first");
+    for (int c : P.first) printf(" %d", c);
+    printf("\nstart_after");
+    for (int c : P.start_after) printf(" %d", c);
+    printf("\n");
+  }
+  const bool whole = feof(f);
+  fclose(f);
+  return whole ? 0 : 2;
+}
diff --git a/include/ocr_hip.h b/include/ocr_hip.h
--- a/include/ocr_hip.h
+++ b/include/ocr_hip.h
@@ -356,6 +356,7 @@
 const char* ocr_pipe_label(ocr_pipe* h, int id);
 int ocr_pipe_det_shape(ocr_pipe* h, int rows, int cols, int* net_rows, int* net_cols);
 int ocr_pipe_stats(ocr_pipe* h, long long out[3]);
+int ocr_pipe_stats_n(ocr_pipe* h, long long* out, int n);
 int ocr_pipe_timing(ocr_pipe* h, int enable);
 int ocr_pipe_timing_filter(ocr_pipe* h, const char* substr);
 int ocr_pipe_timing_report(ocr_pipe* h, char* buf, size_t cap);
```

Result: no change. 1230, median of 5 (+0.0%).
